# stevenlsw/reart

Measured on AMD Instinct MI355X. Metric: relaxation-loop iterations/sec, higher is better.
Workload: dtype f32; 1 GPU; synthetic T=20 x N=4096, P=20, Chamfer+flow, full iteration, one instance/GPU; frames=20, points=4096, parts=20, flow=True, graph=True, steps_per_graph=20, graph_replays=1, eager_steps=0, parallelism=instances x1, instances_per_gpu=1

## Files before the change

reart_amd/csrc/internal.h:

```cpp
#pragma once
#include "common.h"

struct BaseFwdArgs {
    const float *cano;
    const float *W1, *b1, *W2, *p6d, *pt;
    const float *gumbel;
    const float *tau_ptr;
    const int64_t *iter_ptr;
    uint64_t seed;
    float tau;
    int N, P, B, H, Npad;
    float *out;
    float *out_soa;
    int64_t *seg_part;
    float *trans_list;
    float *yT;
    float *hT;
    int *hard_idx;
    float *rt_table;
    float *boxes;
    int pts;
};

struct BaseBwdArgs {
    const float *cano, *W2, *p6d, *pt;
    const float *yT, *hT;
    const float *W1, *b1;
    const int *hard_idx;
    const float *tau_ptr;
    float tau;
    const float *G;
    const float *rt_table;
    const float *gpf;
    int cano_idx;
    int N, P, B, H;
    int nchunk;
    int cpts;
    int dp_sep;
    float *partial;
    const float *step_next;
    float *step_cur;
    float *gW1, *gb1, *gW2, *g6d, *gt;
};

struct AdamSeg { float *p; const float *g; float *m; float *v; int n; float lr; };
struct AdamArgs { AdamSeg seg[8]; int nseg; float beta1, beta2, eps; const int64_t *step_ptr; int step; };

#define REART_BATCH_MAX 6
template <class A>
struct Batched { A a[REART_BATCH_MAX]; };
template <class A>
static inline Batched<A> reart_batched(const A *a, int K) {
    Batched<A> b = {};
    for (int k = 0; k < K && k < REART_BATCH_MAX; ++k) b.a[k] = a[k];
    return b;
}
int reart_base_forward_launch(const BaseFwdArgs *a, int K, hipStream_t st, int force_long);
struct FinalizeAdam {
    int enabled;
    float *W1, *b1, *W2, *p6d, *pt;
    float *m, *v;
    float seg_lr, trans_lr, beta1, beta2, eps;
    float weight_decay;
    const int64_t *step_ptr;
    const float *step;
};

struct StepBook {
    int enabled;
    const double *frame_loss; int n_frame_part;
    const double *flow_part; int n_flow_part;
    int64_t *iter; float *tau; float *losses;
    float *step_next;
    int ring, n_iter;
    float lambda_flow, fixed_tau, end_tau, start_tau, beta1, beta2, seg_lr, trans_lr;
    const double *assign_part; int n_assign_part;
    float *losses_assign;
};
int reart_base_backward_launch(const BaseBwdArgs *args, const FinalizeAdam *adam, const StepBook *book, void *const *workspaces,
                               size_t workspace_bytes, int K, hipStream_t st, int force_long);
int reart_base_forward_long_launch(const BaseFwdArgs *a, int K, hipStream_t st);
int reart_base_backward_long_launch(const BaseBwdArgs *a, int K, hipStream_t st);
int reart_base_bwd_long_tile(int P, int B, int H, int cpts, int *dp_sep, size_t *lds);
#ifdef __HIPCC__
__device__ __forceinline__ float reart_tau_schedule(long cur_iter, int n_iter, float end_t, float start_t) {
    const double c = cos(3.14159265358979323846 * (double)cur_iter / (double)n_iter);
    return (float)((double)end_t + ((double)start_t - (double)end_t) * (c + 1.0) * 0.5);
}
#endif
int reart_adam_ex(const AdamArgs &a, hipStream_t st);

#define PG_SLICES (256 / 12)
int reart_pose_grad_launch(const float *x, const int64_t *part, const float *G, int N, int P, int B, float *partial, hipStream_t st);
int reart_fk_backward_launch(const float *x, const int64_t *part, const float *G, int N, const int32_t *parent,
                             const int32_t *edge_of_part, const int32_t *order, int P, const float *axis, const float *moment,
                             const float *theta, const float *distance, int B, int E, const float *trans, const float *g_trans,
                             float *g_axis, float *g_moment, float *g_theta, float *g_distance, void *workspace,
                             size_t workspace_bytes, hipStream_t st);

int reart_knn_run(int njobs, const float *const *q, const float *const *t,
                  const int64_t *const *lenq, const int64_t *const *lent, int N, const int *P1,
                  const int *P2, int K, int euclidean, float *const *dists, int64_t *const *idx,
                  void *workspace, size_t workspace_bytes, hipStream_t st);

#define NN_BS 64
#define NN_UB 16
struct SoaJob {
    const float *src;
    const int64_t *len;
    float *dst;
    int P, Ppad;
};
struct SoaArgs {
    SoaJob job[2];
};

struct KnnJob {
    const float *q;
    const float *tsoa;
    const int64_t *lenq;
    const int64_t *lent;
    const float *q_alt;
    const int *qmap;
    const int *tlen;
    const float *boxes;
    const int *seed;
    const int *border;
    unsigned int *cost;
    int P1, P2, Ppad, L;
    int nqg;
    float *pd;
    int *pi;
    float *dists;
    int64_t *idx;
};
struct KnnArgs {
    KnnJob job[2];
    int N, S, K, euclidean;
    int items0;
    int items;
};

int reart_knn_launch_slices(const KnnArgs &a, int KK, hipStream_t st);
int reart_soa_launch(const SoaArgs &sa, int maxPpad, int N, int njobs, hipStream_t st);
int reart_knn_pick_split(long waves, int P2, int K);

size_t reart_knn_list_workspace_bytes(int N, int P1, int P2, int K);
int reart_knn_list_run(const float *q, const float *t, const int64_t *lenq, const int64_t *lent, int N, int P1,
                       int P2, int K, int euclidean, float *dists, int64_t *idx, void *workspace,
                       size_t workspace_bytes, hipStream_t st);
template <class T>
int reart_knn_anyd_run(const T *q, const T *t, const int64_t *lenq, const int64_t *lent, int N, int P1, int P2, int D,
                       int K, int euclidean, T *dists, int64_t *idx, void *workspace, size_t workspace_bytes,
                       hipStream_t st);
#ifndef NN_BOX
#define NN_BOX 16
#endif
int reart_boxes_launch(const float *soa, int N, int Ppad, float *boxes, hipStream_t st);
struct SearchArgs {
    KnnJob k1[2]; int n1;
    KnnJob k3;    int n3;
    int G;
    int per;
    int S1, S3;
    int sparse;
    int share;
    int interleave;
    int cloud_resident;
    int cloud_slices;
    int k_nqg;
    unsigned long long *prof;
    unsigned int *prof_pairs;
};
int reart_search_launch(const SearchArgs &a, hipStream_t st);
int reart_search_launch_batch(const SearchArgs *a, int K, hipStream_t st);
int reart_search_grid(int n1, int n3, int G);
int reart_search_grid_cloud(int n1, int n3, int G, int nqg, int slices);
int reart_search_workgroups(const SearchArgs &a);

#ifdef __HIPCC__
__device__ __forceinline__ void reart_top3_insert(float (&kd)[3], int (&ki)[3], float d, int j) {
    const bool l0 = (d < kd[0]) | ((d == kd[0]) & (j < ki[0]));
    const bool l1 = (d < kd[1]) | ((d == kd[1]) & (j < ki[1]));
    const bool l2 = (d < kd[2]) | ((d == kd[2]) & (j < ki[2]));
    kd[2] = l1 ? kd[1] : (l2 ? d : kd[2]);
    ki[2] = l1 ? ki[1] : (l2 ? j : ki[2]);
    kd[1] = l0 ? kd[0] : (l1 ? d : kd[1]);
    ki[1] = l0 ? ki[0] : (l1 ? j : ki[1]);
    kd[0] = l0 ? d : kd[0];
    ki[0] = l0 ? j : ki[0];
}
#endif

struct GridBuildArgs {
    const float *pts;
    const int *offsets;
    int N;
    int stride;
    float *gx, *gy, *gz;
    int *gorig;
    int *cell_start;
    float *meta;
    int *scratch;
};

struct GridQueryArgs {
    const float *q;
    const float *q_alt;
    const int *qmap;
    int nq, E, stride, euclid_unused;
    const float *gx, *gy, *gz;
    const int *gorig, *cell_start;
    const float *meta;
    float *od;
    int *oi;
};

size_t reart_grid_bytes(int E, int stride);
void reart_grid_layout(void *mem, int E, int stride, GridBuildArgs *b);
int reart_grid_build_launch(const GridBuildArgs &b, int E, hipStream_t st);
int reart_grid_query_launch(const GridQueryArgs &q, int K, hipStream_t st);
```

reart_amd/csrc/prune.hip:

```cpp
#include "common.h"
#include "internal.h"
#include <math.h>
#include <string.h>

typedef float f2 __attribute__((ext_vector_type(2)));
#define PR_SMAX 4
#define PR_QCAP 640
#define PR_WPE 6
#define PR_LDS_WAVE_BYTES (64 * 4 + 64 * 16 + 3 * 64 * 8 + PR_QCAP * 4)

#ifdef REART_PRUNE_STATS
__device__ unsigned long long g_prune_stats[8];
extern "C" int reart_debug_prune_stats(unsigned long long *out, int reset) {
    if (hipMemcpyFromSymbol(out, HIP_SYMBOL(g_prune_stats), sizeof(g_prune_stats)) != hipSuccess) return REART_ERR_LAUNCH;
    if (reset) { unsigned long long z[8] = {0}; (void)hipMemcpyToSymbol(HIP_SYMBOL(g_prune_stats), z, sizeof(z)); }
    return REART_OK;
}
#define PRUNE_STAT(k, v) do { if ((threadIdx.x & 63) == 0) atomicAdd(&g_prune_stats[k], (unsigned long long)(v)); } while (0)
#else
#define PRUNE_STAT(k, v) do { } while (0)
#endif
#ifdef REART_PRUNE_PHASE
__device__ unsigned long long g_prune_phase[8];
extern "C" int reart_debug_prune_phase(unsigned long long *out, int reset) {
    if (hipMemcpyFromSymbol(out, HIP_SYMBOL(g_prune_phase), sizeof(g_prune_phase)) != hipSuccess) return REART_ERR_LAUNCH;
    if (reset) { unsigned long long z[8] = {0}; (void)hipMemcpyToSymbol(HIP_SYMBOL(g_prune_phase), z, sizeof(z)); }
    return REART_OK;
}
#define PH_DECL unsigned long long ph_t = __builtin_amdgcn_s_memtime(), ph_acc[7] = {0, 0, 0, 0, 0, 0, 0}
#define PH(k) do { const unsigned long long n_ = __builtin_amdgcn_s_memtime(); ph_acc[k] += n_ - ph_t; ph_t = n_; } while (0)
#define PH_FLUSH(from, to) do { if ((threadIdx.x & 63) == 0) for (int k_ = from; k_ <= to; ++k_) atomicAdd(&g_prune_phase[k_], ph_acc[k_]); } while (0)
#else
#define PH_DECL do { } while (0)
#define PH(k) do { } while (0)
#define PH_FLUSH(from, to) do { } while (0)
#endif

#define PR_WORK(w) ((unsigned)(w) << 20)

#define PR_DPP_OP(NAME, OP, CTRLTXT)                                                                              \
    __device__ __forceinline__ float NAME(float v) {                                                              \
        float r;                                                                                                  \
        asm("s_nop 1\n\t" OP " %0, %1, %1 " CTRLTXT " row_mask:0xf bank_mask:0xf" : "=v"(r) : "v"(v));            \
        return r;                                                                                                 \
    }
PR_DPP_OP(pr_min_q1, "v_min_f32_dpp", "quad_perm:[1,0,3,2]")
PR_DPP_OP(pr_min_q2, "v_min_f32_dpp", "quad_perm:[2,3,0,1]")
PR_DPP_OP(pr_min_hm, "v_min_f32_dpp", "row_half_mirror")
PR_DPP_OP(pr_min_rm, "v_min_f32_dpp", "row_mirror")
PR_DPP_OP(pr_max_q1, "v_max_f32_dpp", "quad_perm:[1,0,3,2]")
PR_DPP_OP(pr_max_q2, "v_max_f32_dpp", "quad_perm:[2,3,0,1]")
PR_DPP_OP(pr_max_hm, "v_max_f32_dpp", "row_half_mirror")
PR_DPP_OP(pr_max_rm, "v_max_f32_dpp", "row_mirror")
__device__ __forceinline__ float pr_row16_min(float v) { return pr_min_rm(pr_min_hm(pr_min_q2(pr_min_q1(v)))); }
__device__ __forceinline__ float pr_row16_max(float v) { return pr_max_rm(pr_max_hm(pr_max_q2(pr_max_q1(v)))); }

__device__ __forceinline__ float rl(float v, int lane) {
    return __int_as_float(__builtin_amdgcn_readlane(__float_as_int(v), lane));
}

__device__ __forceinline__ float box_lb(float lo0, float lo1, float lo2, float hi0, float hi1, float hi2,
                                        float qlo0, float qlo1, float qlo2, float qhi0, float qhi1, float qhi2) {
    const float ex = fmaxf(fmaxf(lo0 - qhi0, qlo0 - hi0), 0.f);
    const float ey = fmaxf(fmaxf(lo1 - qhi1, qlo1 - hi1), 0.f);
    const float ez = fmaxf(fmaxf(lo2 - qhi2, qlo2 - hi2), 0.f);
    return (ex * ex + ey * ey) + ez * ez;
}

template <int KK, bool LDSV, int QCAP, bool BOXL>
__device__ __forceinline__ void knn_pruned_wave(const KnnJob &jb, const int S, const int sparse, const int b, const int g,
                                                const int s, const float *cloud, const int cstride, const float *boxes_p,
                                                float *s_tg, float *s_qc, unsigned int *s_q, float *s_bb, const int share, float *s_xthr,
                                                unsigned long long *s_key, float &qx_o, float &qy_o, float &qz_o,
                                                float (&bm)[KK], int (&bb)[KK], int &work_o, unsigned int &pairs_o) {
    struct { int S, sparse; } a = {S, sparse};
    const int lane = threadIdx.x & 63;
    PH_DECL;

    const int i = g * NN_BS + lane;
    const int ic = i < jb.P1 ? i : jb.P1 - 1;
    const int qb = jb.qmap ? jb.qmap[b] : b;
    const float *qp = (qb < 0 ? jb.q_alt : jb.q + (size_t)qb * jb.P1 * 3) + (size_t)ic * 3;
    const float qx = qp[0], qy = qp[1], qz = qp[2];
    const f2 qx2 = {qx, qx}, qy2 = {qy, qy}, qz2 = {qz, qz};

    const float *tx = cloud;
    const float *ty = tx + cstride;
    const float *tz = ty + cstride;
    const int n2 = jb.tlen ? jb.tlen[b] : jb.P2;
    const int nbox = (n2 + NN_BOX - 1) / NN_BOX;
    const float *bx = boxes_p;

    float thr = 0.f;
    unsigned int wp = 0u;
    {
        const int *sd = jb.seed + ((size_t)b * jb.P1 + ic) * KK;
        int sj[KK];
        bool ok = true;
#pragma unroll
        for (int k = 0; k < KK; ++k) {
            sj[k] = sd[k];
            ok = ok && sj[k] >= 0 && sj[k] < n2;
#pragma unroll
            for (int k2 = 0; k2 < k; ++k2) ok = ok && sj[k] != sj[k2];
        }
        constexpr bool SCR_JOINT = BOXL;
        constexpr bool SCR_FITS = (384 + QCAP + (SCR_JOINT ? 384 : 0)) >= KK * 3 * 64;
        if (SCR_FITS && share) {
            float *s_scr = (float *)s_key;
#pragma unroll
            for (int k = 0; k < KK; ++k) {
                const int j = ok ? sj[k] : 0;
                s_scr[(3 * k + 0) * 64 + lane] = ok ? tx[j] : INFINITY;
                s_scr[(3 * k + 1) * 64 + lane] = ok ? ty[j] : INFINITY;
                s_scr[(3 * k + 2) * 64 + lane] = ok ? tz[j] : INFINITY;
            }
            thr = INFINITY;
            const float *row = s_scr + (lane & 48);
            const bool split = s_xthr != nullptr && a.S > 1;
            const int c0 = split ? 2 * s : 0, cstep = split ? 2 * a.S : 2;
            wp = 64u * KK * 2u * (unsigned)((16 - c0 + cstep - 1) / cstep);
#pragma unroll 1
            for (int c = c0; c < 16; c += cstep) {
                f2 far = {0.f, 0.f};
#pragma unroll
                for (int k = 0; k < KK; ++k) {
                    const f2 dx = qx2 - *(const f2 *)(row + (3 * k + 0) * 64 + c);
                    const f2 dy = qy2 - *(const f2 *)(row + (3 * k + 1) * 64 + c);
                    const f2 dz = qz2 - *(const f2 *)(row + (3 * k + 2) * 64 + c);
                    const f2 d = (dx * dx + dy * dy) + dz * dz;
                    far = f2{fmaxf(far.x, d.x), fmaxf(far.y, d.y)};
                }
                thr = fminf(thr, fminf(far.x, far.y));
            }
            if (split) {
                s_xthr[64 * s + lane] = thr;
                __syncthreads();
                for (int t = 0; t < a.S; ++t) thr = fminf(thr, s_xthr[64 * t + lane]);
            }
            if (!(qx == qx && qy == qy && qz == qz)) thr = INFINITY;
        } else {
#pragma unroll
            for (int k = 0; k < KK; ++k) {
                const int j = ok ? sj[k] : 0;
                thr = fmaxf(thr, reart_sqdist3(qx, qy, qz, tx[j], ty[j], tz[j]));
            }
            wp = 64u * KK;
            if (!ok || !(thr >= 0.f)) thr = INFINITY;
        }
    }

    const float gl0 = pr_row16_min(qx), gl1 = pr_row16_min(qy), gl2 = pr_row16_min(qz);
    const float gh0 = pr_row16_max(qx), gh1 = pr_row16_max(qy), gh2 = pr_row16_max(qz);
    const float gt = pr_row16_max(thr);
    float G[4][7];
#pragma unroll
    for (int q = 0; q < 4; ++q) {
        G[q][0] = rl(gl0, 16 * q); G[q][1] = rl(gl1, 16 * q); G[q][2] = rl(gl2, 16 * q);
        G[q][3] = rl(gh0, 16 * q); G[q][4] = rl(gh1, 16 * q); G[q][5] = rl(gh2, 16 * q);
        G[q][6] = rl(gt, 16 * q);
    }

#pragma unroll
    for (int k = 0; k < KK; ++k) { bm[k] = INFINITY; bb[k] = -1; }
    const float *tx_g = tx;
    wp |= PR_WORK(16);

    const int queue_max = a.sparse;
    int qcnt = 0;
    ((float4 *)s_qc)[lane] = make_float4(qx, qy, qz, 0.f);
    if (KK == 1) s_key[lane] = ~0ull;
    else { s_key[lane] = ~0ull; s_key[64 + lane] = ~0ull; s_key[128 + lane] = ~0ull; }
    auto drain_queue = [&]() {
        for (int e0 = 0; e0 < qcnt; e0 += 64) {
            wp += PR_WORK(6);
            const int e = e0 + lane;
            const bool valid = e < qcnt;
            const unsigned ent = s_q[valid ? e : e0];
            const int ql = (int)(ent & 63u), j0 = (int)(ent >> 6) * NN_BOX;
            wp += (unsigned)__builtin_popcountll(__ballot(valid)) * NN_BOX;
            const float4 qc = ((const float4 *)s_qc)[ql];
            const float *rx = tx_g, *ry = tx_g + cstride, *rz = tx_g + 2 * (size_t)cstride;
            const f2 cx = {qc.x, qc.x}, cy = {qc.y, qc.y}, cz = {qc.z, qc.z};
            float mh[2] = {INFINITY, INFINITY};
#pragma unroll 1
            for (int hf = 0; hf < 2; ++hf) {
                float4 X[2], Y[2], Z[2];
#pragma unroll
                for (int u = 0; u < 2; ++u) {
                    const unsigned ob = 4u * ((unsigned)j0 + 8u * hf + 4u * u);
                    X[u] = *(const float4 *)((const char *)rx + ob);
                    Y[u] = *(const float4 *)((const char *)ry + ob);
                    Z[u] = *(const float4 *)((const char *)rz + ob);
                }
                float m = INFINITY;
#pragma unroll
                for (int u = 0; u < 2; ++u) {
                    const f2 dxa = cx - f2{X[u].x, X[u].y}, dya = cy - f2{Y[u].x, Y[u].y}, dza = cz - f2{Z[u].x, Z[u].y};
                    const f2 dxb = cx - f2{X[u].z, X[u].w}, dyb = cy - f2{Y[u].z, Y[u].w}, dzb = cz - f2{Z[u].z, Z[u].w};
                    const f2 da = (dxa * dxa + dya * dya) + dza * dza;
                    const f2 db = (dxb * dxb + dyb * dyb) + dzb * dzb;
                    m = fminf(fminf(m, fminf(da.x, da.y)), fminf(db.x, db.y));
                }
                if (hf == 0) mh[0] = m; else mh[1] = m;
            }
            if (KK == 1) {
                const float m = fminf(mh[0], mh[1]);
                const unsigned long long key = ((unsigned long long)__float_as_uint(m) << 32) | (unsigned)(j0 + (mh[1] < mh[0] ? 8 : 0));
                if (valid) atomicMin(&s_key[ql], key);
            } else if (valid) {
#pragma unroll
                for (int h = 0; h < 2; ++h) {
                    unsigned long long key = ((unsigned long long)__float_as_uint(mh[h]) << 32) | (unsigned)(j0 + 8 * h);
#pragma unroll
                    for (int lv = 0; lv < 3; ++lv) {
                        const unsigned long long old = atomicMin(&s_key[64 * lv + ql], key);
                        key = old > key ? old : key;
                    }
                }
            }
        }
        qcnt = 0;
        if (KK == 1) {
            const unsigned long long k = s_key[lane];
            const float m = __uint_as_float((unsigned)(k >> 32));
            const int blk = (int)(unsigned)k;
            if (k != ~0ull && ((m < bm[0]) || (m == bm[0] && blk < bb[0]))) { bm[0] = m; bb[0] = blk; }
            thr = fminf(thr, bm[0]);
            s_key[lane] = ~0ull;
        } else {
            float kd[3];
            int ki[3];
#pragma unroll
            for (int c = 0; c < 3; ++c) { kd[c] = bm[c]; ki[c] = bb[c] >= 0 ? bb[c] : 0x7fffffff; }
#pragma unroll
            for (int c = 0; c < 3; ++c) {
                const unsigned long long k = s_key[64 * c + lane];
                s_key[64 * c + lane] = ~0ull;
                if (k != ~0ull) reart_top3_insert(kd, ki, __uint_as_float((unsigned)(k >> 32)), (int)(unsigned)k);
            }
#pragma unroll
            for (int c = 0; c < 3; ++c) { bm[c] = kd[c]; bb[c] = ki[c] == 0x7fffffff ? -1 : ki[c]; }
            thr = fminf(thr, bm[KK - 1]);
        }
    };
    const int per = 64 * a.S;
    PH(0);
    for (int base = 0; base < nbox; base += per) {
        const int bid = base + lane * a.S + s;
        bool pass = false;
        float lo0 = INFINITY, lo1 = INFINITY, lo2 = INFINITY, hi0 = INFINITY, hi1 = INFINITY, hi2 = INFINITY;
        if (bid < nbox) {
            const float4 A = *(const float4 *)(bx + (size_t)bid * 8);
            const float4 Bv = *(const float4 *)(bx + (size_t)bid * 8 + 4);
            lo0 = A.x; lo1 = A.y; lo2 = A.z; hi0 = A.w; hi1 = Bv.x; hi2 = Bv.y;
            if (BOXL) {
                float *o = s_bb + 6 * lane;
                o[0] = lo0; o[1] = lo1; o[2] = lo2; o[3] = hi0; o[4] = hi1; o[5] = hi2;
            }
            const f2 bl0 = {lo0, lo0}, bl1 = {lo1, lo1}, bl2 = {lo2, lo2}, bh0 = {hi0, hi0}, bh1 = {hi1, hi1}, bh2 = {hi2, hi2};
#pragma unroll
            for (int q = 0; q < 4; q += 2) {
                const f2 ql0 = {G[q][0], G[q + 1][0]}, ql1 = {G[q][1], G[q + 1][1]}, ql2 = {G[q][2], G[q + 1][2]};
                const f2 qh0 = {G[q][3], G[q + 1][3]}, qh1 = {G[q][4], G[q + 1][4]}, qh2 = {G[q][5], G[q + 1][5]};
                const f2 a0 = bl0 - qh0, c0 = ql0 - bh0, a1 = bl1 - qh1, c1 = ql1 - bh1, a2 = bl2 - qh2, c2 = ql2 - bh2;
                const f2 e0 = {fmaxf(fmaxf(a0.x, c0.x), 0.f), fmaxf(fmaxf(a0.y, c0.y), 0.f)};
                const f2 e1 = {fmaxf(fmaxf(a1.x, c1.x), 0.f), fmaxf(fmaxf(a1.y, c1.y), 0.f)};
                const f2 e2 = {fmaxf(fmaxf(a2.x, c2.x), 0.f), fmaxf(fmaxf(a2.y, c2.y), 0.f)};
                const f2 lb = (e0 * e0 + e1 * e1) + e2 * e2;
                pass = pass || (lb.x <= G[q][6]) || (lb.y <= G[q + 1][6]);
            }
        }
        unsigned long long mask = __ballot(pass);
        PH(1);
        PRUNE_STAT(KK == 1 ? 0 : 3, 0);
        if (KK == 1) PRUNE_STAT(1, __builtin_popcountll(mask));
        if (KK == 1) PRUNE_STAT(3, __builtin_popcountll(__ballot(thr == INFINITY)));
        auto scan_box = [&](const int bit) {
            wp += PR_WORK(5) | (64u * NN_BOX);
            if (KK == 1) PRUNE_STAT(2, 1);
            const int j0 = (base + bit * a.S + s) * NN_BOX;
            if (!LDSV) {
                const int l = lane < 48 ? lane : 47;
                const float v = tx_g[(size_t)(l >> 4) * cstride + j0 + (l & 15)];
                if (lane < 48) s_tg[lane] = v;
            }
            const float *tx = LDSV ? tx_g : s_tg - j0;
            const float *ty = tx + (LDSV ? cstride : 16), *tz = ty + (LDSV ? cstride : 16);
            if (KK == 1) {
                float mh[2] = {INFINITY, INFINITY};
#pragma unroll
                for (int u = 0; u < NN_BOX; u += 2) {
                    const f2 dx = qx2 - *(const f2 *)(tx + j0 + u);
                    const f2 dy = qy2 - *(const f2 *)(ty + j0 + u);
                    const f2 dz = qz2 - *(const f2 *)(tz + j0 + u);
                    const f2 d = (dx * dx + dy * dy) + dz * dz;
                    mh[u >> 3] = fminf(fminf(mh[u >> 3], d.x), d.y);
                }
                const float m = fminf(mh[0], mh[1]);
                if (m < bm[0]) { bm[0] = m; bb[0] = j0 + (mh[1] < mh[0] ? 8 : 0); }
                thr = fminf(thr, m);
            } else {
                constexpr int UBK = 8;
#pragma unroll
                for (int h = 0; h < NN_BOX; h += UBK) {
                    float m = INFINITY;
#pragma unroll
                    for (int u = 0; u < UBK; u += 2) {
                        const f2 dx = qx2 - *(const f2 *)(tx + j0 + h + u);
                        const f2 dy = qy2 - *(const f2 *)(ty + j0 + h + u);
                        const f2 dz = qz2 - *(const f2 *)(tz + j0 + h + u);
                        const f2 d = (dx * dx + dy * dy) + dz * dz;
                        m = fminf(fminf(m, d.x), d.y);
                    }
#pragma unroll
                    for (int c = KK - 1; c >= 0; --c) {
                        const int cp = c > 0 ? c - 1 : 0;
                        const bool lt_prev = (c > 0) && (m < bm[cp]);
                        const bool lt_cur = m < bm[c];
                        bm[c] = lt_prev ? bm[cp] : (lt_cur ? m : bm[c]);
                        bb[c] = lt_prev ? bb[cp] : (lt_cur ? j0 + h : bb[c]);
                    }
                }
                thr = fminf(thr, bm[KK - 1]);
            }
        };
        auto enqueue_box = [&](const int bit, const unsigned long long need, const bool nd, const int nneed) {
            wp += PR_WORK(1);
            if (KK == 1) PRUNE_STAT(2, 1);
            const int bid = base + bit * a.S + s;
            const int rank = __builtin_amdgcn_mbcnt_hi((unsigned)(need >> 32), __builtin_amdgcn_mbcnt_lo((unsigned)need, 0u));
            if (nd) s_q[qcnt + rank] = ((unsigned)bid << 6) | (unsigned)lane;
            qcnt += nneed;
        };
        while (mask) {
            unsigned long long cm = mask;
            mask = 0ull;
            while (cm) {
            const int bA = __builtin_ctzll(cm);
            cm &= cm - 1;
            const bool hasB = cm != 0;
            const int bB = hasB ? __builtin_ctzll(cm) : bA;
            if (hasB) cm &= cm - 1;
            f2 L0, L1, L2, H0, H1, H2;
            if (BOXL) {
                const float *pA = s_bb + 6 * bA, *pB = s_bb + 6 * bB;
                L0 = f2{pA[0], pB[0]}; L1 = f2{pA[1], pB[1]}; L2 = f2{pA[2], pB[2]};
                H0 = f2{pA[3], pB[3]}; H1 = f2{pA[4], pB[4]}; H2 = f2{pA[5], pB[5]};
            } else {
                L0 = f2{rl(lo0, bA), rl(lo0, bB)}; L1 = f2{rl(lo1, bA), rl(lo1, bB)}; L2 = f2{rl(lo2, bA), rl(lo2, bB)};
                H0 = f2{rl(hi0, bA), rl(hi0, bB)}; H1 = f2{rl(hi1, bA), rl(hi1, bB)}; H2 = f2{rl(hi2, bA), rl(hi2, bB)};
            }
            const f2 a0 = L0 - qx2, c0 = qx2 - H0, a1 = L1 - qy2, c1 = qy2 - H1, a2 = L2 - qz2, c2 = qz2 - H2;
            const f2 e0 = {fmaxf(fmaxf(a0.x, c0.x), 0.f), fmaxf(fmaxf(a0.y, c0.y), 0.f)};
            const f2 e1 = {fmaxf(fmaxf(a1.x, c1.x), 0.f), fmaxf(fmaxf(a1.y, c1.y), 0.f)};
            const f2 e2 = {fmaxf(fmaxf(a2.x, c2.x), 0.f), fmaxf(fmaxf(a2.y, c2.y), 0.f)};
            const f2 lb = (e0 * e0 + e1 * e1) + e2 * e2;
            wp += PR_WORK(2);
            PH(2);
#pragma unroll 1
            for (int h = 0; h < (hasB ? 2 : 1); ++h) {
                const float lbh = h ? lb.y : lb.x;
#ifdef REART_PRUNE_STATS
                if (KK == 1) {
                    const int nl = __builtin_popcountll(__ballot(lbh <= thr));
                    if (nl) PRUNE_STAT(nl == 1 ? 4 : (nl < 4 ? 5 : (nl < 8 ? 6 : 7)), 1);
                }
#endif
                const bool nd = lbh <= thr;
                const unsigned long long need = __ballot(nd);
                if (need) {
                    const int nneed = __builtin_popcountll(need);
                    if (nneed <= queue_max) {
                        enqueue_box(h ? bB : bA, need, nd, nneed);
                        PH(4);
                        if (qcnt > QCAP - 64) { drain_queue(); PH(5); }
                    } else {
                        scan_box(h ? bB : bA);
                        PH(3);
                    }
                }
            }
            }
        }
    }

    PH(2);
    if (qcnt > 0) drain_queue();
    PH(5);
    PH_FLUSH(0, 5);
    qx_o = qx; qy_o = qy; qz_o = qz;
    work_o = (int)(wp >> 20); pairs_o = wp & 0xFFFFFu;
}


template <bool BATCH>
__global__ __launch_bounds__(64 * PR_SMAX, PR_WPE) void knn_group_kernel(Batched<SearchArgs> ab) {
    const SearchArgs &a = ab.a[BATCH ? blockIdx.y : 0];
    extern __shared__ __attribute__((aligned(16))) unsigned char s_dyn[];
#define PARK_M(t) ((float *)(s_dyn + (size_t)(t) * PR_LDS_WAVE_BYTES + 64 * 4 + 64 * 16))
#define PARK_B(t) ((int *)(s_dyn + (size_t)(t) * PR_LDS_WAVE_BYTES + 64 * 4 + 64 * 16 + 3 * 64 * 4))
    __shared__ unsigned int s_wk[PR_SMAX][2];
    __shared__ float s_xthr[PR_SMAX][64];
    __shared__ unsigned int s_ticket;
    __shared__ unsigned long long s_t0;
    if (threadIdx.x == 0) { s_ticket = 0u; s_t0 = a.prof ? wall_clock64() : 0ull; }
    __syncthreads();
    const int L = blockIdx.x, x = L & 7, r = L >> 3;
    const int s = threadIdx.x >> 6, lane = threadIdx.x & 63;
    const unsigned long long t0 = s_t0;
    const int items1 = a.n1 * a.per, items3 = a.n3 * a.per;
    const int mixed = (a.n1 == 2 && a.n3) ? 3 * a.per : 0;
    int kind, idx;
    if (r < mixed) {
        const int q = r / 3, rr = r - 3 * q;
        kind = rr < 2 ? 1 : 3;
        idx = rr < 2 ? 2 * q + rr : q;
    } else {
        const int d1 = mixed ? 2 * a.per : 0, d3 = mixed ? a.per : 0;
        const int v = r - mixed, left1 = items1 - d1;
        kind = v < left1 ? 1 : 3;
        idx = v < left1 ? d1 + v : d3 + (v - left1);
    }
    const int j = kind == 1 ? (a.n1 == 2 ? (idx & 1) : 0) : 0;
    const int p = kind == 1 ? (a.n1 == 2 ? (idx >> 1) : idx) : idx;
    const int pos = a.interleave ? p * 8 + x : x * a.per + p;
    const bool live = p < a.per && pos < a.G && (kind == 1 ? idx < items1 : idx < items3);
    if (!live) {
        if (a.prof && threadIdx.x == 0) { a.prof[2 * (size_t)L] = t0; a.prof[2 * (size_t)L + 1] = t0; a.prof_pairs[L] = 0u; }
        return;
    }
    const KnnJob &jb = kind == 1 ? a.k1[j] : a.k3;
    const int S = kind == 1 ? a.S1 : a.S3;
    if (s >= S) return;
    const int grp = jb.border ? jb.border[pos] : pos;
    const int b = grp / jb.nqg, g = grp - b * jb.nqg;
    float qx = 0.f, qy = 0.f, qz = 0.f;
    float bm[3] = {INFINITY, INFINITY, INFINITY};
    int bb[3] = {-1, -1, -1};
    int work = 0;
    unsigned int pairs = 0u;
    {
        unsigned char *wl = s_dyn + (size_t)s * PR_LDS_WAVE_BYTES;
        float *s_tg = (float *)wl;
        float *s_qc = (float *)(wl + 64 * 4);
        unsigned long long *s_key = (unsigned long long *)(wl + 64 * 4 + 64 * 16);
        unsigned int *s_q = (unsigned int *)(wl + 64 * 4 + 64 * 16 + 3 * 64 * 8);
        static_assert(384 + PR_QCAP >= 3 * 3 * 64, "neighbour seeds of a K = 3 item: 9 x 64 floats in the result slots + the queue's space");
        static_assert(PR_QCAP >= 384 + 128, "box bounds of a coarse round + at least two drain steps of queue");
        float *s_bb = (float *)s_q;
        s_q += 384;
        constexpr int QC = PR_QCAP - 384;
        const float *cloud = jb.tsoa + (size_t)b * 3 * jb.Ppad;
        const float *boxes_p = jb.boxes + (size_t)b * (jb.Ppad / NN_BOX) * 8;
        if (kind == 1) {
            float m1[1]; int b1[1];
            knn_pruned_wave<1, false, QC, true>(jb, S, a.sparse, b, g, s, cloud, jb.Ppad, boxes_p, s_tg, s_qc, s_q, s_bb, a.share, a.share > 1 ? &s_xthr[0][0] : nullptr, s_key,
                                               qx, qy, qz, m1, b1, work, pairs);
            bm[0] = m1[0]; bb[0] = b1[0];
        } else {
            knn_pruned_wave<3, false, QC, true>(jb, S, a.sparse, b, g, s, cloud, jb.Ppad, boxes_p, s_tg, s_qc, s_q, s_bb, a.share, a.share > 1 ? &s_xthr[0][0] : nullptr, s_key,
                                               qx, qy, qz, bm, bb, work, pairs);
        }
    }
    if (S > 1) {
#pragma unroll
        for (int k = 0; k < 3; ++k) { PARK_M(s)[k * 64 + lane] = bm[k]; PARK_B(s)[k * 64 + lane] = bb[k]; }
        if (lane == 0) { s_wk[s][0] = (unsigned int)work; s_wk[s][1] = pairs; }
        __threadfence_block();
        int ticket = 0;
        if (lane == 0) ticket = (int)atomicAdd(&s_ticket, 1u);
        ticket = __builtin_amdgcn_readfirstlane(ticket);
#ifdef REART_PRUNE_PHASE
        if (lane == 0) atomicAdd(&g_prune_phase[7], 1ull);
#endif
        if (ticket != S - 1) return;
        __threadfence_block();
        work = 0; pairs = 0u;
        for (int t = 0; t < S; ++t) { work += (int)s_wk[t][0]; pairs += s_wk[t][1]; }
#pragma unroll
        for (int k = 0; k < 3; ++k) { bm[k] = PARK_M(0)[k * 64 + lane]; bb[k] = PARK_B(0)[k * 64 + lane]; }
    }
    const int i = g * NN_BS + lane;
    const float *tx = jb.tsoa + (size_t)b * 3 * jb.Ppad, *ty = tx + jb.Ppad, *tz = ty + jb.Ppad;
    if (kind == 1) {
        float m = bm[0];
        int blk = bb[0];
        for (int t = 1; t < S; ++t) {
            const float mt = PARK_M(t)[lane];
            const int bt = PARK_B(t)[lane];
            const bool take = bt >= 0 && ((mt < m) || (mt == m && (blk < 0 || bt < blk)));
            m = take ? mt : m; blk = take ? bt : blk;
        }
        int bi = 0x7fffffff;
        if (blk >= 0) {
#pragma unroll
            for (int u = NN_BOX / 2 - 1; u >= 0; --u) {
                const float d = reart_sqdist3(qx, qy, qz, tx[blk + u], ty[blk + u], tz[blk + u]);
                if (d == m) bi = blk + u;
            }
        }
        pairs += 64u * (NN_BOX / 2);
        if (i < jb.P1) {
            const size_t o = (size_t)b * jb.P1 + i;
            jb.pd[o] = m; jb.pi[o] = bi;
        }
    } else {
        float kd[3] = {INFINITY, INFINITY, INFINITY};
        int ki[3] = {0x7fffffff, 0x7fffffff, 0x7fffffff};
#pragma unroll
        for (int k = 0; k < 3; ++k) reart_top3_insert(kd, ki, bm[k], bb[k] >= 0 ? bb[k] : 0x7fffffff);
        for (int t = 1; t < S; ++t) {
#pragma unroll
            for (int k = 0; k < 3; ++k) {
                const int bt = PARK_B(t)[k * 64 + lane];
                reart_top3_insert(kd, ki, PARK_M(t)[k * 64 + lane], bt >= 0 ? bt : 0x7fffffff);
            }
        }
        if (i < jb.P1) {
            const size_t o = ((size_t)b * jb.P1 + i) * 3;
#pragma unroll
            for (int k = 0; k < 3; ++k) { jb.pd[o + k] = kd[k]; jb.pi[o + k] = kd[k] < INFINITY ? ki[k] : -1; }
        }
    }
    if (lane == 0) {
        if (jb.cost) jb.cost[pos] = (unsigned int)work;
        if (a.prof) {
            a.prof[2 * (size_t)L] = t0; a.prof[2 * (size_t)L + 1] = wall_clock64();
            a.prof_pairs[L] = pairs;
        }
    }
}

#define PC_WAVES 16
#define PC_QCAP 256
#define PC_WAVE_BYTES (64 * 16 + 3 * 64 * 8 + PC_QCAP * 4)
__global__ __launch_bounds__(64 * PC_WAVES) void knn_cloud_kernel(SearchArgs a) {
    extern __shared__ __attribute__((aligned(16))) unsigned char s_dyn[];
    const int L = blockIdx.x, w = threadIdx.x >> 6, lane = threadIdx.x & 63;
    unsigned long long t0 = 0ull;
    if (a.prof && threadIdx.x == 0) t0 = wall_clock64();
    const int njobs = a.n1 + a.n3;
    const int jsel = L % njobs;
    const int rest = L / njobs;
    const int B = a.G / a.k_nqg;
    const int b = rest % B, blk = rest / B;
    const int kind = jsel < a.n1 ? 1 : 3;
    const KnnJob &jb = kind == 1 ? a.k1[jsel] : a.k3;
    const int S = a.cloud_slices, gpw = PC_WAVES / S;
    const int Ppad = jb.Ppad, nboxp = Ppad / NN_BOX;
    float *cl = (float *)s_dyn;
    float *bxs = cl + 3 * (size_t)Ppad;
    {
        const float4 *src = (const float4 *)(jb.tsoa + (size_t)b * 3 * Ppad);
        float4 *dst = (float4 *)cl;
        const int n4 = 3 * Ppad / 4;
        for (int e = threadIdx.x; e < n4; e += 64 * PC_WAVES) dst[e] = src[e];
        const float4 *sb = (const float4 *)(jb.boxes + (size_t)b * nboxp * 8);
        float4 *db = (float4 *)bxs;
        for (int e = threadIdx.x; e < 2 * nboxp; e += 64 * PC_WAVES) db[e] = sb[e];
    }
    __syncthreads();
    const int g = blk * gpw + w / S, sl = w % S;
    unsigned int pairs = 0u;
    int work = 0;
    unsigned char *wbase = s_dyn + (size_t)(3 * Ppad + 8 * nboxp) * 4;
    unsigned long long *s_key = (unsigned long long *)(wbase + (size_t)w * PC_WAVE_BYTES + 64 * 16);
    float qx = 0.f, qy = 0.f, qz = 0.f;
    float bm[3] = {INFINITY, INFINITY, INFINITY};
    int bb[3] = {-1, -1, -1};
    if (g < jb.nqg) {
        unsigned char *wl = wbase + (size_t)w * PC_WAVE_BYTES;
        float *s_qc = (float *)wl;
        unsigned int *s_q = (unsigned int *)(wl + 64 * 16 + 3 * 64 * 8);
        if (kind == 1) {
            float m1[1]; int b1[1];
            knn_pruned_wave<1, true, PC_QCAP, false>(jb, S, a.sparse, b, g, sl, cl, Ppad, bxs, nullptr, s_qc, s_q, nullptr, a.share, nullptr, s_key, qx, qy, qz,
                                              m1, b1, work, pairs);
            bm[0] = m1[0]; bb[0] = b1[0];
        } else {
            knn_pruned_wave<3, true, PC_QCAP, false>(jb, S, a.sparse, b, g, sl, cl, Ppad, bxs, nullptr, s_qc, s_q, nullptr, a.share, nullptr, s_key, qx, qy, qz,
                                              bm, bb, work, pairs);
        }
        if (S > 1 && sl > 0) {
#pragma unroll
            for (int k = 0; k < 3; ++k)
                s_key[64 * k + lane] = bb[k] >= 0 ? (((unsigned long long)__float_as_uint(bm[k]) << 32) | (unsigned)bb[k]) : ~0ull;
            if (lane == 0) { s_key[192] = (unsigned long long)(unsigned)work; s_key[193] = (unsigned long long)pairs; }
        }
    }
    if (S > 1) __syncthreads();
    if (g < jb.nqg && sl == 0) {
        for (int t = 1; t < S; ++t) {
            const unsigned long long *ok = (const unsigned long long *)(wbase + (size_t)(w + t) * PC_WAVE_BYTES + 64 * 16);
            work += (int)(unsigned)ok[192]; pairs += (unsigned)ok[193];
            if (kind == 1) {
                const unsigned long long k = ok[lane];
                const float m = __uint_as_float((unsigned)(k >> 32));
                const int bt = (int)(unsigned)k;
                if (k != ~0ull && ((m < bm[0]) || (m == bm[0] && (bb[0] < 0 || bt < bb[0])))) { bm[0] = m; bb[0] = bt; }
            } else {
                float kd[3];
                int ki[3];
#pragma unroll
                for (int c = 0; c < 3; ++c) { kd[c] = bm[c]; ki[c] = bb[c] >= 0 ? bb[c] : 0x7fffffff; }
#pragma unroll
                for (int c = 0; c < 3; ++c) {
                    const unsigned long long k = ok[64 * c + lane];
                    if (k != ~0ull) reart_top3_insert(kd, ki, __uint_as_float((unsigned)(k >> 32)), (int)(unsigned)k);
                }
#pragma unroll
                for (int c = 0; c < 3; ++c) { bm[c] = kd[c]; bb[c] = ki[c] == 0x7fffffff ? -1 : ki[c]; }
            }
        }
        const int i = g * NN_BS + lane;
        if (kind == 1) {
            int bi = 0x7fffffff;
            if (bb[0] >= 0) {
                const float *tx = cl, *ty = cl + Ppad, *tz = cl + 2 * (size_t)Ppad;
#pragma unroll
                for (int u = NN_BOX / 2 - 1; u >= 0; --u) {
                    const float d = reart_sqdist3(qx, qy, qz, tx[bb[0] + u], ty[bb[0] + u], tz[bb[0] + u]);
                    if (d == bm[0]) bi = bb[0] + u;
                }
            }
            pairs += 64u * (NN_BOX / 2);
            if (i < jb.P1) {
                const size_t o = (size_t)b * jb.P1 + i;
                jb.pd[o] = bm[0]; jb.pi[o] = bi;
            }
        } else if (i < jb.P1) {
            const size_t o = ((size_t)b * jb.P1 + i) * 3;
#pragma unroll
            for (int k = 0; k < 3; ++k) { jb.pd[o + k] = bm[k]; jb.pi[o + k] = bm[k] < INFINITY ? bb[k] : -1; }
        }
        if (lane == 0 && jb.cost) jb.cost[b * jb.nqg + g] = (unsigned int)work;
    } else {
        pairs = 0u;
    }
    if (a.prof) {
        __shared__ unsigned int s_pairs[PC_WAVES];
        if (lane == 0) s_pairs[w] = pairs;
        __syncthreads();
        if (threadIdx.x == 0) {
            unsigned int tot = 0u;
            for (int k = 0; k < PC_WAVES; ++k) tot += s_pairs[k];
            a.prof[2 * (size_t)L] = t0; a.prof[2 * (size_t)L + 1] = wall_clock64();
            a.prof_pairs[L] = tot;
        }
    }
}

static size_t search_cloud_lds(const SearchArgs &a) {
    int Ppad = 0;
    for (int j = 0; j < a.n1; ++j) Ppad = a.k1[j].Ppad > Ppad ? a.k1[j].Ppad : Ppad;
    if (a.n3) Ppad = a.k3.Ppad > Ppad ? a.k3.Ppad : Ppad;
    const size_t need = (size_t)(3 * Ppad + 8 * (Ppad / NN_BOX)) * 4 + (size_t)PC_WAVES * PC_WAVE_BYTES + 256;
    return need <= 152 * 1024 ? need : 0;
}

static int search_check(SearchArgs &a) {
    if (a.n1 < 0 || a.n1 > 2 || a.n3 < 0 || a.n3 > 1 || a.n1 + a.n3 == 0 || a.G < 1) return REART_ERR_INVALID_ARG;
    if ((a.n1 && (a.S1 < 1 || a.S1 > PR_SMAX)) || (a.n3 && (a.S3 < 1 || a.S3 > PR_SMAX))) return REART_ERR_INVALID_ARG;
    for (int j = 0; j < a.n1; ++j)
        if (!a.k1[j].boxes || !a.k1[j].seed || !a.k1[j].pd || !a.k1[j].pi) return REART_ERR_INVALID_ARG;
    if (a.n3 && (!a.k3.boxes || !a.k3.seed || !a.k3.pd || !a.k3.pi)) return REART_ERR_INVALID_ARG;
    a.per = reart_div_up(a.G, 8);
    a.k_nqg = a.n1 ? a.k1[0].nqg : a.k3.nqg;
    return REART_OK;
}

int reart_search_launch(const SearchArgs &a_in, hipStream_t st) {
    SearchArgs a = a_in;
    const int rc = search_check(a);
    if (rc != REART_OK) return rc;
    const size_t cl_lds = a.cloud_resident ? search_cloud_lds(a) : 0;
    a.cloud_slices = (a.cloud_slices == 1 || a.cloud_slices == 2 || a.cloud_slices == 4 || a.cloud_slices == 8) ? a.cloud_slices : 4;
    if (cl_lds) {
        if (hipFuncSetAttribute((const void *)knn_cloud_kernel, hipFuncAttributeMaxDynamicSharedMemorySize, 152 * 1024) != hipSuccess)
            return REART_ERR_LAUNCH;
        hipLaunchKernelGGL(knn_cloud_kernel, dim3(reart_search_grid_cloud(a.n1, a.n3, a.G, a.k_nqg, a.cloud_slices)), dim3(64 * PC_WAVES),
                           cl_lds, st, a);
        REART_CHECK_LAUNCH();
        return REART_OK;
    }
    return reart_search_launch_batch(&a, 1, st);
}
int reart_search_launch_batch(const SearchArgs *ak, int K, hipStream_t st) {
    if (K < 1 || K > REART_BATCH_MAX) return REART_ERR_INVALID_ARG;
    Batched<SearchArgs> ab = {};
    for (int k = 0; k < K; ++k) {
        ab.a[k] = ak[k];
        const int rc = search_check(ab.a[k]);
        if (rc != REART_OK) return rc;
        const SearchArgs &a = ab.a[k], &a0 = ab.a[0];
        if (a.n1 != a0.n1 || a.n3 != a0.n3 || a.G != a0.G || a.S1 != a0.S1 || a.S3 != a0.S3) return REART_ERR_INVALID_ARG;
    }
    const SearchArgs &a = ab.a[0];
    const int S = (a.n1 ? a.S1 : 0) > (a.n3 ? a.S3 : 0) ? a.S1 : a.S3;
    const size_t lds = (size_t)S * PR_LDS_WAVE_BYTES;
    if (K == 1) hipLaunchKernelGGL(knn_group_kernel<false>, dim3(reart_search_grid(a.n1, a.n3, a.G)), dim3(64 * S), lds, st, ab);
    else hipLaunchKernelGGL(knn_group_kernel<true>, dim3(reart_search_grid(a.n1, a.n3, a.G), K), dim3(64 * S), lds, st, ab);
    REART_CHECK_LAUNCH();
    return REART_OK;
}
int reart_search_workgroups(const SearchArgs &a) {
    const int nqg = a.n1 ? a.k1[0].nqg : a.k3.nqg;
    const int cs = (a.cloud_slices == 1 || a.cloud_slices == 2 || a.cloud_slices == 4 || a.cloud_slices == 8) ? a.cloud_slices : 4;
    if (a.cloud_resident && search_cloud_lds(a)) return reart_search_grid_cloud(a.n1, a.n3, a.G, nqg, cs);
    return reart_search_grid(a.n1, a.n3, a.G);
}
int reart_search_grid(int n1, int n3, int G) { return 8 * (n1 + n3) * reart_div_up(G, 8); }
int reart_search_grid_cloud(int n1, int n3, int G, int nqg, int slices) {
    return (n1 + n3) * (G / nqg) * reart_div_up(nqg, PC_WAVES / slices);
}

template <int KK>
__global__ __launch_bounds__(256) void knn_warm_finish_kernel(KnnArgs a) {
    const KnnJob jb = a.job[0];
    const int b = blockIdx.y, i = blockIdx.x * 256 + threadIdx.x;
    if (i >= jb.P1) return;
    float kd[KK];
    int ki[KK];
#pragma unroll
    for (int k = 0; k < KK; ++k) { kd[k] = INFINITY; ki[k] = 0x7fffffff; }
    auto insert = [&](float d, int j) {
#pragma unroll
        for (int s = KK - 1; s >= 0; --s) {
            const int sp = s > 0 ? s - 1 : 0;
            const bool lp = (s > 0) && ((d < kd[sp]) | ((d == kd[sp]) & (j < ki[sp])));
            const bool lc = (d < kd[s]) | ((d == kd[s]) & (j < ki[s]));
            kd[s] = lp ? kd[sp] : (lc ? d : kd[s]);
            ki[s] = lp ? ki[sp] : (lc ? j : ki[s]);
        }
    };
    {
        const size_t o = ((size_t)b * jb.P1 + i) * KK;
#pragma unroll
        for (int k = 0; k < KK; ++k) {
            const float d = jb.pd[o + k];
            const int q = jb.pi[o + k];
            insert(d, (d < INFINITY && q >= 0) ? q : 0x7fffffff);
        }
    }
    if (KK > 1) {
        const float *qp = jb.q + ((size_t)b * jb.P1 + i) * 3;
        const float qx = qp[0], qy = qp[1], qz = qp[2];
        const float *tx = jb.tsoa + (size_t)b * 3 * jb.Ppad, *ty = tx + jb.Ppad, *tz = ty + jb.Ppad;
        int blk[KK];
#pragma unroll
        for (int k = 0; k < KK; ++k) { blk[k] = kd[k] < INFINITY ? ki[k] : -1; kd[k] = INFINITY; ki[k] = 0x7fffffff; }
#pragma unroll
        for (int c = 0; c < KK; ++c) {
            if (blk[c] < 0) continue;
            for (int u = 0; u < 8; ++u) {
                const int jj = blk[c] + u;
                const float d = reart_sqdist3(qx, qy, qz, tx[jj], ty[jj], tz[jj]);
                insert(d, d < INFINITY ? jj : 0x7fffffff);
            }
        }
    }
    const int n2 = jb.P2;
    const int valid = KK < n2 ? KK : n2;
#pragma unroll
    for (int k = 0; k < KK; ++k) {
        const bool ok = k < valid && ki[k] != 0x7fffffff;
        const size_t o = ((size_t)b * jb.P1 + i) * KK + k;
        jb.dists[o] = ok ? kd[k] : 0.0f;
        jb.idx[o] = ok ? (int64_t)ki[k] : (int64_t)0;
        ((int *)jb.seed)[o] = ok ? ki[k] : -1;
    }
}

struct WarmPlan { int S, Ppad; size_t o_soa, o_box, o_pd, o_pi, total; };
static int warm_plan(int N, int P1, int P2, int K, WarmPlan *p) {
    if (N < 0 || P1 < 0 || P2 < 0 || (K != 1 && K != 3)) return REART_ERR_INVALID_ARG;
    p->S = 4;
    while (p->S > 1 && reart_div_up(P2, p->S) < 64) p->S -= 1;
    p->Ppad = (int)reart_align_up((size_t)(P2 > 0 ? P2 : 1), NN_BOX);
    reart_arena ws;
    p->o_soa = ws.take_bytes(sizeof(float) * 3 * (size_t)N * p->Ppad);
    p->o_box = ws.take_bytes(sizeof(float) * 8 * (size_t)N * (p->Ppad / NN_BOX));
    p->o_pd = ws.take_bytes(sizeof(float) * (size_t)N * P1 * K);
    p->o_pi = ws.take_bytes(sizeof(int) * (size_t)N * P1 * K);
    p->total = ws.off;
    return REART_OK;
}

extern "C" size_t reart_knn_points_warm_workspace_bytes(int N, int P1, int P2, int K) {
    WarmPlan p;
    return warm_plan(N, P1, P2, K, &p) == REART_OK ? p.total : 0;
}

extern "C" int reart_knn_points_idx_warm(const float *p1, const float *p2, int N, int P1, int P2, int K,
                                         int32_t *seed, float *dists, int64_t *idx, void *workspace,
                                         size_t workspace_bytes, void *stream) {
    WarmPlan p;
    int rc = warm_plan(N, P1, P2, K, &p);
    if (rc != REART_OK) return rc;
    if (N == 0 || P1 == 0) return REART_OK;
    if (!p1 || !p2 || !seed || !dists || !idx || P2 < 1) return REART_ERR_INVALID_ARG;
    if (!workspace || workspace_bytes < p.total) return REART_ERR_INVALID_ARG;
    hipStream_t st = (hipStream_t)stream;
    char *ws = (char *)workspace;
    SoaArgs sa = {};
    for (int j = 0; j < 2; ++j) {
        sa.job[j].src = p2; sa.job[j].len = nullptr; sa.job[j].dst = (float *)(ws + p.o_soa);
        sa.job[j].P = P2; sa.job[j].Ppad = p.Ppad;
    }
    rc = reart_soa_launch(sa, p.Ppad, N, 1, st);
    if (rc != REART_OK) return rc;
    rc = reart_boxes_launch((const float *)(ws + p.o_soa), N, p.Ppad, (float *)(ws + p.o_box), st);
    if (rc != REART_OK) return rc;
    KnnArgs a = {};
    a.N = N; a.S = p.S; a.K = K; a.euclidean = 0;
    KnnJob &jb = a.job[0];
    jb.q = p1; jb.tsoa = (const float *)(ws + p.o_soa); jb.boxes = (const float *)(ws + p.o_box);
    jb.seed = seed; jb.P1 = P1; jb.P2 = P2; jb.Ppad = p.Ppad; jb.L = 0; jb.nqg = reart_div_up(P1, NN_BS);
    jb.pd = (float *)(ws + p.o_pd); jb.pi = (int *)(ws + p.o_pi); jb.dists = dists; jb.idx = idx;
    a.job[1] = jb;
    SearchArgs sr = {};
    sr.G = N * jb.nqg; sr.S1 = sr.S3 = p.S; sr.sparse = 40; sr.share = 2;
    if (K == 1) { sr.k1[0] = jb; sr.n1 = 1; } else { sr.k3 = jb; sr.n3 = 1; }
    rc = reart_search_launch(sr, st);
    if (rc != REART_OK) return rc;
    const dim3 fg(reart_div_up(P1, 256), N);
    if (K == 1) hipLaunchKernelGGL((knn_warm_finish_kernel<1>), fg, dim3(256), 0, st, a);
    else hipLaunchKernelGGL((knn_warm_finish_kernel<3>), fg, dim3(256), 0, st, a);
    REART_CHECK_LAUNCH();
    return REART_OK;
}
```

reart_amd/csrc/step.hip:

```cpp
#include "common.h"
#include "internal.h"
#include "blocksort.h"
#include "consumer_dev.h"
#include "flow_dev.h"
#include <math.h>
#include <string.h>

struct StepPlan {
    int S1, L1, Npad;
    int S3, Mpad;
    int nchunk, nparams;
    size_t o_ysoa, o_xsoa, o_rsoa, o_rlen, o_qmap;
    size_t o_pd0, o_pi0, o_pd1, o_pi1, o_pd3, o_pi3;
    size_t o_yT, o_hT, o_hard, o_rt, o_G, o_gpf, o_fx, o_floss, o_apart, o_fpart, o_grads, o_bwd;
    size_t o_bc;
    size_t o_ticket;
    size_t o_boxY, o_boxX, o_boxR;
    int keep_hT;
    int pruned;
    int W1, W3;
    int sparse;
    size_t o_seed3;
    size_t o_border;
    size_t o_cost;
    size_t o_prof, o_prof_pairs, o_prof_acc;
    size_t o_gridY, o_gridR;
    int gstrideY, gstrideR;
    size_t bwd_bytes, total;
};

#define FLOW_BS 256
#define CG_BS 1024
#define POST_FBS 512
#define CG_RANGE 1024
static_assert(CG_BS == CG_RANGE, "chamfer_grad_kernel: thread tid owns target r0 + tid");

static int step_plan(const reart_relax_config *c, StepPlan *p) {
    if (c->N <= 0 || c->P <= 0 || c->P > 32 || c->B <= 0 || c->H <= 0) return REART_ERR_INVALID_ARG;
    if (c->use_flow && (c->flow_k != 3 || c->M_max < 3)) return REART_ERR_UNSUPPORTED;
    const long waves1 = 2L * c->B * reart_div_up(c->N, NN_BS);
    p->pruned = (c->use_boxes && !c->use_grid && c->search_mode != 1) ? 1 : 0;
    p->W1 = (c->tune_slices >= 1 && c->tune_slices <= 4) ? c->tune_slices : 3;
    p->W3 = (c->tune_slices_flow >= 1 && c->tune_slices_flow <= 4) ? c->tune_slices_flow : p->W1;
    p->sparse = c->tune_sparse < 0 ? 0 : (c->tune_sparse == 0 ? 40 : (c->tune_sparse > 64 ? 64 : c->tune_sparse));
    p->S1 = p->pruned ? 1 : reart_knn_pick_split(waves1, c->N, 1);
    p->L1 = (int)reart_align_up((size_t)reart_div_up(c->N, p->S1), NN_BOX);
    p->Npad = p->L1 * p->S1;
    p->S3 = 1; p->Mpad = 0;
    if (c->use_flow) {
        const long waves3 = (long)c->B * reart_div_up(c->N, NN_BS);
        p->S3 = p->pruned ? 1 : reart_knn_pick_split(waves3, c->M_max, 3);
        p->Mpad = (int)reart_align_up((size_t)reart_div_up(c->M_max, p->S3), NN_BOX) * p->S3;
    }
    p->nchunk = reart_div_up(c->N, 64);
    p->nparams = 3 * c->H + c->H + c->P * c->H + 6 * c->B * c->P + 3 * c->B * c->P;
    reart_arena ws;
    const size_t BN = (size_t)c->B * c->N;
    p->o_ysoa = ws.take_bytes(sizeof(float) * 3 * c->B * (size_t)p->Npad);
    p->o_xsoa = ws.take_bytes(sizeof(float) * 3 * c->B * (size_t)p->Npad);
    p->o_rsoa = ws.take_bytes(sizeof(float) * 3 * c->B * (size_t)p->Mpad);
    p->o_rlen = ws.take_bytes(sizeof(int) * c->B);
    p->o_qmap = ws.take_bytes(sizeof(int) * (c->B + 1));
    p->o_pd0 = ws.take_bytes(sizeof(float) * p->S1 * BN);
    p->o_pi0 = ws.take_bytes(sizeof(int) * p->S1 * BN);
    p->o_pd1 = ws.take_bytes(sizeof(float) * p->S1 * BN);
    p->o_pi1 = ws.take_bytes(sizeof(int) * p->S1 * BN);
    p->o_pd3 = ws.take_bytes(c->use_flow ? sizeof(float) * p->S3 * BN * 3 : 0);
    p->o_pi3 = ws.take_bytes(c->use_flow ? sizeof(int) * p->S3 * BN * 3 : 0);
    p->o_yT = ws.take_bytes(sizeof(float) * (size_t)c->P * c->N);
    p->keep_hT = (c->tune_long > 0 || reart_base_path(c->P, c->B, c->H, 0) != 0 || reart_base_path(c->P, c->B, c->H, 1) != 0) ? 1 : 0;
    p->o_hT = ws.take_bytes(p->keep_hT ? sizeof(float) * (size_t)c->H * c->N : 0);
    p->o_hard = ws.take_bytes(sizeof(int) * (size_t)c->N);
    p->o_rt = ws.take_bytes(sizeof(float) * 12 * (size_t)c->B * c->P);
    p->o_G = ws.take_bytes(sizeof(float) * 3 * BN);
    p->o_gpf = ws.take_bytes(sizeof(float) * 3 * BN);
    p->o_fx = ws.take_bytes(sizeof(double));
    p->o_floss = ws.take_bytes(sizeof(double) * (size_t)c->B * reart_div_up(c->N, CG_RANGE));
    p->o_apart = ws.take_bytes(c->recon_with_assign ? sizeof(double) * (size_t)c->B * reart_div_up(c->N, CG_RANGE) : 0);
    p->o_fpart = ws.take_bytes(sizeof(double) * (size_t)c->B * reart_div_up(c->N, FLOW_BS));
    p->o_grads = ws.take_bytes(sizeof(float) * p->nparams);
    p->bwd_bytes = reart_base_backward_workspace_bytes(c->N, c->P, c->B, c->H);
    p->o_bwd = ws.take_bytes(p->bwd_bytes);
    p->o_bc = ws.take_bytes(8 * sizeof(float));
    p->o_ticket = ws.take_bytes(4 * sizeof(unsigned int));
    p->o_boxY = ws.take_bytes(sizeof(float) * 8 * (size_t)c->B * (p->Npad / NN_BOX));
    p->o_boxX = ws.take_bytes(sizeof(float) * 8 * (size_t)c->B * (p->Npad / NN_BOX));
    p->o_boxR = ws.take_bytes(sizeof(float) * 8 * (size_t)c->B * (p->Mpad / NN_BOX + 1));
    p->o_seed3 = ws.take_bytes((p->pruned && c->use_flow) ? sizeof(int) * BN * 3 : 0);
    const size_t G = (size_t)c->B * reart_div_up(c->N, NN_BS);
    p->o_border = ws.take_bytes(sizeof(int) * 3 * G);
    p->o_cost = ws.take_bytes(sizeof(unsigned int) * 3 * G);
    const size_t nprof = (c->profile && p->pruned) ? (size_t)reart_search_grid(2, 1, (int)G) : 0;
    p->o_prof = ws.take_bytes(sizeof(unsigned long long) * 2 * nprof);
    p->o_prof_pairs = ws.take_bytes(sizeof(unsigned int) * nprof);
    p->o_prof_acc = ws.take_bytes(sizeof(unsigned long long) * 4);
    p->gstrideY = (int)reart_align_up((size_t)c->N, 64);
    p->gstrideR = (int)reart_align_up((size_t)(c->M_max > 0 ? c->M_max : 1), 64);
    p->o_gridY = ws.take_bytes(c->use_grid ? reart_grid_bytes(c->B, p->gstrideY) : 0);
    p->o_gridR = ws.take_bytes((c->use_grid && c->use_flow) ? reart_grid_bytes(c->B, p->gstrideR) : 0);
    p->total = ws.off;
    return REART_OK;
}

extern "C" size_t reart_relax_workspace_bytes(const reart_relax_config *cfg) {
    StepPlan p;
    if (!cfg || step_plan(cfg, &p) != REART_OK) return 0;
    return p.total;
}

__global__ void relax_init_kernel(reart_relax_config c, const int *__restrict__ ref_off,
                                  int *__restrict__ rlen, int *__restrict__ qmap,
                                  int64_t *__restrict__ iter, float *__restrict__ tau,
                                  const float *__restrict__ pc_list, int *__restrict__ fx_bits,
                                  float *__restrict__ adam_step, int *__restrict__ seed3, int *__restrict__ border) {
    __shared__ float s_max[1024];
    const int t = threadIdx.x;
    if (seed3)
        for (size_t e = t; e < (size_t)c.B * c.N * 3; e += 1024) seed3[e] = (int)(e % 3);
    float mx = 0.f;
    for (size_t e = t; e < (size_t)c.B * c.N * 3; e += 1024) mx = fmaxf(mx, fabsf(pc_list[e]));
    s_max[t] = mx;
    __syncthreads();
    for (int o = 512; o >= 1; o >>= 1) {
        if (t < o) s_max[t] = fmaxf(s_max[t], s_max[t + o]);
        __syncthreads();
    }
    if (t == 0) {
        const double bound = 8.0 * (double)c.N * fmax((double)s_max[0], 1e-30);
        int bits = (int)floor(61.0 - log2(bound));
        fx_bits[0] = bits > 39 ? 39 : (bits < 0 ? 0 : bits);
    }
    if (t < c.B) {
        {
            const int nqg = (c.N + NN_BS - 1) / NN_BS, ng = c.B * nqg;
            for (int g = 0; g < nqg; ++g)
                for (int j = 0; j < 3; ++j) border[j * ng + t * nqg + g] = t * nqg + g;
        }
        qmap[t] = (t < c.cano_idx) ? t : (t == c.cano_idx ? -1 : t - 1);
        if (c.use_flow) rlen[t] = ref_off[t + 1] - ref_off[t];
    }
    if (t == 0) {
        const long it = (long)iter[0];
        tau[0] = c.fixed_tau > 0.f ? c.fixed_tau : reart_tau_schedule(it + 1, c.n_iter, c.end_tau, c.start_tau);
        const double bc1 = 1.0 - pow((double)c.beta1, (double)(it + 1));
        const double bc2 = sqrt(1.0 - pow((double)c.beta2, (double)(it + 1)));
        for (int s = 0; s < 8; s += 4) {
            adam_step[s] = (float)((double)c.seg_lr / bc1);
            adam_step[s + 1] = (float)((double)c.trans_lr / bc1);
            adam_step[s + 2] = (float)bc2;
            adam_step[s + 3] = 0.f;
        }
    }
}

__global__ __launch_bounds__(256) void ref_soa_kernel(const float *__restrict__ ref_loc,
                                                      const int *__restrict__ ref_off, int Mpad,
                                                      float *__restrict__ soa) {
    const int f = blockIdx.y, j = blockIdx.x * 256 + threadIdx.x;
    if (j >= Mpad) return;
    const int o = ref_off[f], m = ref_off[f + 1] - o;
    float x = INFINITY, y = INFINITY, z = INFINITY;
    if (j < m) {
        const float *p = ref_loc + 3 * ((size_t)o + j);
        x = p[0]; y = p[1]; z = p[2];
    }
    float *d = soa + (size_t)f * 3 * Mpad;
    d[j] = x; d[Mpad + j] = y; d[2 * (size_t)Mpad + j] = z;
}

extern "C" int reart_relax_prepare(const reart_relax_config *cfg, const reart_relax_buffers *bufs,
                                   void *workspace, size_t workspace_bytes, void *stream) {
    StepPlan p;
    if (!cfg || !bufs) return REART_ERR_INVALID_ARG;
    int rc = step_plan(cfg, &p);
    if (rc != REART_OK) return rc;
    if (!workspace || workspace_bytes < p.total) return REART_ERR_INVALID_ARG;
    if (!bufs->cano || !bufs->pc_list || !bufs->iter || !bufs->tau) return REART_ERR_INVALID_ARG;
    if (cfg->use_flow && (!bufs->ref_loc || !bufs->ref_flow || !bufs->ref_off)) return REART_ERR_INVALID_ARG;
    static_assert(REART_MAX_POSE_LEN <= 1024, "relax_init_kernel: one thread per frame");
    if (cfg->B > REART_MAX_POSE_LEN) return REART_ERR_UNSUPPORTED;
    char *ws = (char *)workspace;
    hipStream_t st = (hipStream_t)stream;
    SoaArgs sa = {};
    for (int j = 0; j < 2; ++j) {
        sa.job[j].src = bufs->pc_list; sa.job[j].len = nullptr;
        sa.job[j].dst = (float *)(ws + p.o_ysoa); sa.job[j].P = cfg->N; sa.job[j].Ppad = p.Npad;
    }
    rc = reart_soa_launch(sa, p.Npad, cfg->B, 1, st);
    if (rc != REART_OK) return rc;
    hipLaunchKernelGGL(relax_init_kernel, dim3(1), dim3(1024), 0, st, *cfg, bufs->ref_off,
                       (int *)(ws + p.o_rlen), (int *)(ws + p.o_qmap), bufs->iter, bufs->tau, bufs->pc_list,
                       (int *)(ws + p.o_fx), (float *)(ws + p.o_bc),
                       (p.pruned && cfg->use_flow) ? (int *)(ws + p.o_seed3) : nullptr, (int *)(ws + p.o_border));
    if (hipMemsetAsync(ws + p.o_ticket, 0, 4 * sizeof(unsigned int), st) != hipSuccess) return REART_ERR_LAUNCH;
    if (hipMemsetAsync(ws + p.o_prof_acc, 0, 4 * sizeof(unsigned long long), st) != hipSuccess) return REART_ERR_LAUNCH;
    if (p.pruned) {
        if (hipMemsetAsync(ws + p.o_pi0, 0, sizeof(int) * (size_t)cfg->B * cfg->N, st) != hipSuccess) return REART_ERR_LAUNCH;
        if (hipMemsetAsync(ws + p.o_pi1, 0, sizeof(int) * (size_t)cfg->B * cfg->N, st) != hipSuccess) return REART_ERR_LAUNCH;
    }
    rc = reart_boxes_launch((const float *)(ws + p.o_ysoa), cfg->B, p.Npad, (float *)(ws + p.o_boxY), st);
    if (rc != REART_OK) return rc;
    if (cfg->use_grid) {
        GridBuildArgs gb = {};
        reart_grid_layout(ws + p.o_gridY, cfg->B, p.gstrideY, &gb);
        gb.pts = bufs->pc_list; gb.offsets = nullptr; gb.N = cfg->N;
        rc = reart_grid_build_launch(gb, cfg->B, st);
        if (rc != REART_OK) return rc;
        if (cfg->use_flow) {
            GridBuildArgs gr = {};
            reart_grid_layout(ws + p.o_gridR, cfg->B, p.gstrideR, &gr);
            gr.pts = bufs->ref_loc; gr.offsets = bufs->ref_off; gr.N = cfg->M_max;
            rc = reart_grid_build_launch(gr, cfg->B, st);
            if (rc != REART_OK) return rc;
        }
    }
    if (cfg->use_flow)
    {
        hipLaunchKernelGGL(ref_soa_kernel, dim3(reart_div_up(p.Mpad, 256), cfg->B), dim3(256), 0, st,
                           bufs->ref_loc, bufs->ref_off, p.Mpad, (float *)(ws + p.o_rsoa));
        rc = reart_boxes_launch((const float *)(ws + p.o_rsoa), cfg->B, p.Mpad, (float *)(ws + p.o_boxR), st);
        if (rc != REART_OK) return rc;
    }
    REART_CHECK_LAUNCH();
    return REART_OK;
}

struct FlowArgs {
    const float *pd; const int *pi;
    const float *ref_flow; const int *ref_off; const int *qmap;
    const float *X; const float *cano;
    int N, B, S, euclidean, robust, cano_idx;
    int blocks;
    const float *rsoa; int Mpad;
    float smooth, lambda;
    float *gpf;
    double *part;
    int *seed_out;
};

template <int SL, int FBS>
__device__ __forceinline__ void flow_blend_body(const FlowArgs &a, const int bx, const int f, const int nbx) {
    __shared__ double s_red[FBS / REART_WAVE];
    const int n = bx * FBS + threadIdx.x;
    double term = 0.0;
    if (n < a.N) {
        constexpr int NU = SL == 1 ? 1 : 4;
        float kd[3] = {INFINITY, INFINITY, INFINITY};
        int ki[3] = {0x7fffffff, 0x7fffffff, 0x7fffffff};
        const size_t stride = (size_t)a.B * a.N * 3, o0 = ((size_t)f * a.N + n) * 3;
        const float *c0 = reart_complete_frame(a.X, a.cano, a.N, a.cano_idx, f) + 3 * (size_t)n;
        const float *c1 = reart_complete_frame(a.X, a.cano, a.N, a.cano_idx, f + 1) + 3 * (size_t)n;
        const float c0v[3] = {c0[0], c0[1], c0[2]}, c1v[3] = {c1[0], c1[1], c1[2]};
        const int roff = a.ref_off[f];
        for (int s0 = 0; s0 < (SL ? 1 : a.S); s0 += 4) {
            float e[NU][3];
            int q[NU][3];
#pragma unroll
            for (int u = 0; u < NU; ++u) {
                const bool ok = s0 + u < a.S;
                const size_t o = o0 + (size_t)(ok ? s0 + u : 0) * stride;
#pragma unroll
                for (int k = 0; k < 3; ++k) { e[u][k] = a.pd[o + k]; q[u][k] = a.pi[o + k]; }
                if (!ok) { e[u][0] = INFINITY; e[u][1] = INFINITY; e[u][2] = INFINITY; }
            }
#pragma unroll
            for (int u = 0; u < NU; ++u)
#pragma unroll
                for (int k = 0; k < 3; ++k)
                    reart_top3_insert(kd, ki, e[u][k], e[u][k] < INFINITY ? q[u][k] : 0x7fffffff);
        }
        if (a.blocks) {
            const float *tx = a.rsoa + (size_t)f * 3 * a.Mpad, *ty = tx + a.Mpad, *tz = ty + a.Mpad;
            int bb[3], nv[3];
#pragma unroll
            for (int cb = 0; cb < 3; ++cb) {
                bb[cb] = (kd[cb] < INFINITY) ? ki[cb] : -1;
                nv[cb] = bb[cb] < 0 ? 0 : 8;
            }
            reart_rescan3(c0v, tx, ty, tz, bb, nv, kd, ki);
        }
#pragma unroll
        for (int k = 0; k < 3; ++k) ki[k] = ki[k] == 0x7fffffff ? 0 : ki[k];
        if (a.seed_out) {
            int *so = a.seed_out + 3 * ((size_t)f * a.N + n);
            so[0] = ki[0]; so[1] = ki[1]; so[2] = ki[2];
        }
        const float *rf = a.ref_flow + 3 * (size_t)roff;
        float rfl[3][3];
#pragma unroll
        for (int k = 0; k < 3; ++k)
#pragma unroll
            for (int c = 0; c < 3; ++c) rfl[k][c] = rf[3 * (size_t)ki[k] + c];
        float w[3], wsum = 0.f, dmin = INFINITY, fmx = -INFINITY;
#pragma unroll
        for (int k = 0; k < 3; ++k) {
            float d = a.euclidean ? sqrtf(kd[k]) : kd[k];
            if (d < 1e-10f) d = 1e-10f;
            w[k] = 1.0f / d;
            wsum += w[k];
            dmin = fminf(dmin, d);
            fmx = fmaxf(fmx, (rfl[k][0] * rfl[k][0] + rfl[k][1] * rfl[k][1]) + rfl[k][2] * rfl[k][2]);
        }
        float gtf[3] = {0.f, 0.f, 0.f};
#pragma unroll
        for (int k = 0; k < 3; ++k) {
            const float wn = w[k] / wsum;
            gtf[0] += rfl[k][0] * wn; gtf[1] += rfl[k][1] * wn; gtf[2] += rfl[k][2] * wn;
        }
        const bool m = (dmin <= fmx) || (dmin <= 0.05f);
        float fl = 0.f, sm = 0.f;
        float *go = a.gpf + 3 * ((size_t)f * a.N + n);
#pragma unroll
        for (int c = 0; c < 3; ++c) {
            const float p = c1v[c] - c0v[c];
            const float d = p - gtf[c];
            fl += a.robust ? huber1(d) : d * d;
            sm += p * p;
            const float gf = a.robust ? huber1_grad(d) : 2.0f * d;
            go[c] = a.lambda * (m ? gf : a.smooth * (2.0f * p));
        }
        term = m ? (double)fl : (double)(a.smooth * sm);
    }
    term = reart_block_sum_d<FBS>(term, s_red);
    if (threadIdx.x == 0) a.part[(size_t)f * nbx + bx] = term;
}

struct CGradArgs {
    const float *X, *Y;
    const float *pd0; const int *pi0;
    const float *pd1; const int *pi1;
    const int *fx_bits;
    int N, B, S0, S1;
    float *G;
    double *loss_part;
    int *seed0, *seed1;
    const int *map;
    double *assign_part;
    float lambda;
};
template <int SL>
__device__ __forceinline__ void merge_slices(const float *__restrict__ pd, const int *__restrict__ pi, int S,
                                             size_t stride, size_t o0, int nmax, float &d, int &j) {
    d = INFINITY; j = 0x7fffffff;
    constexpr int NU = SL == 1 ? 1 : 4;
    for (int s0 = 0; s0 < (SL ? 1 : S); s0 += 4) {
        float e[NU];
        int q[NU];
#pragma unroll
        for (int u = 0; u < NU; ++u) {
            const size_t o = o0 + (size_t)(s0 + u < S ? s0 + u : S - 1) * stride;
            e[u] = pd[o]; q[u] = pi[o];
        }
#pragma unroll
        for (int u = 0; u < NU; ++u) {
            const bool l = (e[u] < d) | ((e[u] == d) & (q[u] < j));
            d = l ? e[u] : d; j = l ? q[u] : j;
        }
    }
    j = j < 0 ? 0 : (j >= nmax ? nmax - 1 : j);
}

template <int SL, bool AS>
__device__ __forceinline__ void chamfer_grad_body(const CGradArgs &a, const int bx, const int b, const int nbx) {
    __shared__ unsigned long long s_acc[CG_RANGE * 3];
    __shared__ double s_red[CG_BS / REART_WAVE];
    const int tid = threadIdx.x, N = a.N;
    const int r0 = bx * CG_RANGE;
    const float *x = a.X + (size_t)b * N * 3, *y = a.Y + (size_t)b * N * 3;
    const size_t stride = (size_t)a.B * N, ob = (size_t)b * N;
    for (int e = tid; e < CG_RANGE * 3; e += CG_BS) s_acc[e] = 0ull;
    const int io = r0 + tid, ioc = io < N ? io : N - 1;
    float d0;
    int j0;
    int am = -1;
    if (AS) am = a.map[ob + ioc];
    merge_slices<SL>(a.pd0, a.pi0, a.S0, stride, ob + ioc, N, d0, j0);
    const int sbits = a.fx_bits[0];
    float yn[3], xo[3];
#pragma unroll
    for (int k = 0; k < 3; ++k) { yn[k] = y[3 * j0 + k]; xo[k] = x[3 * ioc + k]; }
    const bool paired = AS && am >= 0 && am < N;
    float ya[3] = {0.f, 0.f, 0.f};
    if (AS) {
        const int amc = paired ? am : 0;
#pragma unroll
        for (int k = 0; k < 3; ++k) ya[k] = y[3 * amc + k];
    }
    __syncthreads();
    float d1own = 0.f;
    constexpr int IL = 4;
    for (int ib = tid; ib < N; ib += IL * CG_BS) {
        float d1[IL];
        int j1[IL];
#pragma unroll
        for (int u = 0; u < IL; ++u) {
            const int i = ib + u * CG_BS;
            merge_slices<SL>(a.pd1, a.pi1, a.S1, stride, ob + (i < N ? i : N - 1), N, d1[u], j1[u]);
        }
        float df[IL][3];
#pragma unroll
        for (int u = 0; u < IL; ++u) {
            const int i = ib + u * CG_BS;
            const int ic = i < N ? i : N - 1;
#pragma unroll
            for (int k = 0; k < 3; ++k) df[u][k] = x[3 * j1[u] + k] - y[3 * ic + k];
        }
#pragma unroll
        for (int u = 0; u < IL; ++u) {
            const int i = ib + u * CG_BS;
            if (i >= N) continue;
            if (i == io) {
                d1own = d1[u];
                if (a.seed1) a.seed1[ob + i] = j1[u];
            }
            const int jl = j1[u] - r0;
            if (jl >= 0 && jl < CG_RANGE) {
#pragma unroll
                for (int k = 0; k < 3; ++k)
                    atomicAdd(&s_acc[3 * jl + k], (unsigned long long)reart_fixed_from_float(df[u][k], sbits));
            }
        }
    }
    if (io < N && a.seed0) a.seed0[ob + io] = j0;
    __syncthreads();
    double term = 0.0, aterm = 0.0;
    if (io < N) {
        term = (double)(d0 + d1own);
        const double inv2 = 2.0 * exp2((double)-sbits);
        float *G = a.G + 3 * (ob + io);
        float sq = 0.f;
#pragma unroll
        for (int k = 0; k < 3; ++k) {
            const float gc = 2.0f * (xo[k] - yn[k]) + (float)((double)(long long)s_acc[3 * tid + k] * inv2);
            if (AS && paired) {
                const float d = xo[k] - ya[k];
                sq += d * d;
                G[k] = gc + a.lambda * (2.0f * d);
            } else {
                G[k] = gc;
            }
        }
        if (AS && paired) aterm = (double)sq;
    }
    term = reart_block_sum_d<CG_BS>(term, s_red);
    if (tid == 0) a.loss_part[(size_t)b * nbx + bx] = term;
    if (AS) {
        __syncthreads();
        aterm = reart_block_sum_d<CG_BS>(aterm, s_red);
        if (tid == 0) a.assign_part[(size_t)b * nbx + bx] = aterm * (double)a.lambda;
    }
}

template <int SL, bool BATCH, bool AS>
__global__ __launch_bounds__(CG_BS) void chamfer_grad_kernel(Batched<CGradArgs> ab) {
    chamfer_grad_body<SL, AS>(ab.a[BATCH ? blockIdx.z : 0], blockIdx.x, blockIdx.y, gridDim.x);
}
template <int SL, bool BATCH>
__global__ __launch_bounds__(FLOW_BS) void flow_blend_kernel(Batched<FlowArgs> ab) {
    flow_blend_body<SL, FLOW_BS>(ab.a[BATCH ? blockIdx.z : 0], blockIdx.x, blockIdx.y, gridDim.x);
}
struct OrderArgs {
    const unsigned int *cost[3];
    int *border[3];
    int groups;
    int per;
    const unsigned long long *prof; const unsigned int *prof_pairs; unsigned long long *prof_acc; int nprof;
};
#define ORD_MAX 4
__device__ __forceinline__ void order_body(const OrderArgs &o, const int j) {
    __shared__ unsigned int s_hist[8 * 256];
    const int tid = threadIdx.x;
    if (!o.cost[j] || o.groups > ORD_MAX * CG_BS) return;
    for (int e = tid; e < 8 * 256; e += CG_BS) s_hist[e] = 0u;
    __syncthreads();
    int old[ORD_MAX], bucket[ORD_MAX];
#pragma unroll
    for (int u = 0; u < ORD_MAX; ++u) {
        const int k = tid + u * CG_BS;
        old[u] = 0; bucket[u] = -1;
        if (k < o.groups) {
            const unsigned int c = o.cost[j][k] >> 5;
            old[u] = o.border[j][k];
            bucket[u] = (k / o.per) * 256 + 255 - (int)(c < 255u ? c : 255u);
            atomicAdd(&s_hist[bucket[u]], 1u);
        }
    }
    __syncthreads();
    for (int c0 = (tid >> 6); c0 < 8; c0 += CG_BS / 64) {
        const int l = tid & 63;
        unsigned int v[4], sum = 0u;
#pragma unroll
        for (int k = 0; k < 4; ++k) { v[k] = s_hist[c0 * 256 + 4 * l + k]; sum += v[k]; }
        unsigned int incl = sum;
#pragma unroll
        for (int off = 1; off < 64; off <<= 1) {
            const unsigned int t = __shfl_up(incl, off, 64);
            if (l >= off) incl += t;
        }
        unsigned int run = (unsigned int)(c0 * o.per) + (incl - sum);
#pragma unroll
        for (int k = 0; k < 4; ++k) { s_hist[c0 * 256 + 4 * l + k] = run; run += v[k]; }
    }
    __syncthreads();
#pragma unroll
    for (int u = 0; u < ORD_MAX; ++u)
        if (bucket[u] >= 0) o.border[j][atomicAdd(&s_hist[bucket[u]], 1u)] = old[u];
}
__device__ __forceinline__ void prof_body(const OrderArgs &o) {
    __shared__ unsigned long long s_lo[CG_BS / 64], s_hi[CG_BS / 64], s_sum[CG_BS / 64], s_busy[CG_BS / 64];
    const int tid = threadIdx.x;
    unsigned long long lo = ~0ull, hi = 0ull, sum = 0ull, busy = 0ull;
    for (int k = tid; k < o.nprof; k += CG_BS) {
        const unsigned long long a = o.prof[2 * (size_t)k], b = o.prof[2 * (size_t)k + 1];
        lo = a < lo ? a : lo; hi = b > hi ? b : hi; sum += o.prof_pairs[k]; busy += b - a;
    }
#pragma unroll
    for (int off = 32; off >= 1; off >>= 1) {
        const unsigned long long l2 = __shfl_xor(lo, off, 64), h2 = __shfl_xor(hi, off, 64), s2 = __shfl_xor(sum, off, 64);
        const unsigned long long b2 = __shfl_xor(busy, off, 64);
        lo = l2 < lo ? l2 : lo; hi = h2 > hi ? h2 : hi; sum += s2; busy += b2;
    }
    if ((tid & 63) == 0) { s_lo[tid >> 6] = lo; s_hi[tid >> 6] = hi; s_sum[tid >> 6] = sum; s_busy[tid >> 6] = busy; }
    __syncthreads();
    if (tid == 0) {
        for (int w = 1; w < CG_BS / 64; ++w) {
            lo = s_lo[w] < lo ? s_lo[w] : lo; hi = s_hi[w] > hi ? s_hi[w] : hi; sum += s_sum[w]; busy += s_busy[w];
        }
        o.prof_acc[0] += 1ull; o.prof_acc[1] += hi - lo; o.prof_acc[2] += sum; o.prof_acc[3] += busy;
    }
}
struct PostArgs { int nfx, nflow, ncx, nwork, norder; FlowArgs fl; CGradArgs cg; OrderArgs od; };
#ifdef REART_PHASE_CLOCK
__device__ unsigned long long g_post_ts[8];
extern "C" int reart_debug_post_clock(unsigned long long *out) {
    return hipMemcpyFromSymbol(out, HIP_SYMBOL(g_post_ts), sizeof(g_post_ts)) == hipSuccess ? REART_OK : REART_ERR_LAUNCH;
}
#define POST_TS(k) do { __syncthreads(); if (threadIdx.x == 0 && blockIdx.y == 0) g_post_ts[k] = __builtin_amdgcn_s_memtime(); } while (0)
#else
#define POST_TS(k) do { } while (0)
#endif
template <bool BATCH, bool AS>
__global__ __launch_bounds__(CG_BS) void post_kernel(Batched<PostArgs> ab) {
    const PostArgs &a = ab.a[BATCH ? blockIdx.y : 0];
    const int w = blockIdx.x;
    if (w < a.nflow) {
        if (threadIdx.x >= POST_FBS) return;
        if (w == 1) POST_TS(0);
        flow_blend_body<1, POST_FBS>(a.fl, w % a.nfx, w / a.nfx, a.nfx);
        if (w == 1) POST_TS(1);
    } else if (w < a.nwork) {
        if (w == a.nflow + 1) POST_TS(2);
        chamfer_grad_body<1, AS>(a.cg, (w - a.nflow) % a.ncx, (w - a.nflow) / a.ncx, a.ncx);
        if (w == a.nflow + 1) POST_TS(3);
    } else if (w < a.nwork + a.norder) {
        if (w == a.nwork) POST_TS(4);
        order_body(a.od, w - a.nwork);
        if (w == a.nwork) POST_TS(5);
    } else {
        POST_TS(6);
        prof_body(a.od);
        POST_TS(7);
    }
}

struct AssignArgs {
    const float *X, *Y;
    const int *map;
    int N, B;
    float lambda;
    float *G;
    double *loss_part;
};
__device__ __forceinline__ void assign_grad_body(const AssignArgs &a, int bx, int b, int gx) {
    __shared__ double s_red[CG_BS / REART_WAVE];
    const int i = bx * CG_BS + threadIdx.x, tid = threadIdx.x;
    double term = 0.0;
    if (i < a.N) {
        const size_t o = (size_t)b * a.N + i;
        const int m = a.map[o];
        float g[3] = {0.f, 0.f, 0.f};
        if (m >= 0 && m < a.N) {
            float sq = 0.f;
#pragma unroll
            for (int k = 0; k < 3; ++k) {
                const float d = a.X[3 * o + k] - a.Y[3 * ((size_t)b * a.N + m) + k];
                sq += d * d;
                g[k] = a.lambda * (2.0f * d);
            }
            term = (double)sq;
        }
#pragma unroll
        for (int k = 0; k < 3; ++k) a.G[3 * o + k] = g[k];
    }
    term = reart_block_sum_d<CG_BS>(term, s_red);
    if (tid == 0) a.loss_part[(size_t)b * gx + bx] = term * (double)a.lambda;
}
template <bool BATCH>
__global__ __launch_bounds__(CG_BS) void assign_grad_kernel(Batched<AssignArgs> ab) {
    assign_grad_body(ab.a[BATCH ? blockIdx.z : 0], blockIdx.x, blockIdx.y, gridDim.x);
}

#define MARK(k) do { if (ev) (void)hipEventRecord(ev[k], st); } while (0)

struct StepGeom {
    int pruned, grid;
    int flow;
    int merged;
    int has_search;
    int static_order;
    int has_fl, has_aa, has_cg;
    int fl_sl, cg_sl;
    int fgx, fgy, ncg, post_blocks, N, B;
    int long_model;
    int cg_assign;
};
struct StepLaunch {
    StepGeom g;
    BaseFwdArgs fa; SearchArgs sa; KnnArgs ka, k3; GridQueryArgs gq3, gq1; PostArgs pa;
    FlowArgs fl; AssignArgs aa; CGradArgs cg;
    BaseBwdArgs ba; FinalizeAdam ad; StepBook bk; void *ws_bwd; size_t bwd_bytes;
    int auto_s1, auto_s3;
    void *aux_stream, *ev_fork, *ev_join;
};

static int step_describe(const reart_relax_config *cfg, const reart_relax_buffers *bufs, void *workspace, size_t workspace_bytes,
                         bool forward_only, StepLaunch *out) {
    StepPlan p;
    if (!cfg || !bufs) return REART_ERR_INVALID_ARG;
    int rc = step_plan(cfg, &p);
    if (rc != REART_OK) return rc;
    if (!workspace || workspace_bytes < p.total) return REART_ERR_INVALID_ARG;
    if (!bufs->W1 || !bufs->b1 || !bufs->W2 || !bufs->p6d || !bufs->pt || !bufs->adam_m || !bufs->adam_v ||
        !bufs->pc_trans || !bufs->iter || !bufs->tau)
        return REART_ERR_INVALID_ARG;
    const reart_relax_config &c = *cfg;
    StepLaunch &L = *out;
    L = StepLaunch{};
    StepGeom &g = L.g;
    char *ws = (char *)workspace;
    const int N = c.N, B = c.B, P = c.P, H = c.H;
    float *G = (float *)(ws + p.o_G);
    g.N = N; g.B = B; g.pruned = p.pruned; g.grid = c.use_grid ? 1 : 0; g.flow = c.use_flow ? 1 : 0;
    g.long_model = c.tune_long > 0 ? 1 : 0;

    BaseFwdArgs &fa = L.fa;
    fa.cano = bufs->cano; fa.W1 = bufs->W1; fa.b1 = bufs->b1; fa.W2 = bufs->W2; fa.p6d = bufs->p6d;
    fa.pt = bufs->pt; fa.gumbel = bufs->gumbel; fa.tau_ptr = bufs->tau; fa.iter_ptr = bufs->iter;
    fa.seed = c.seed; fa.tau = 1.0f; fa.N = N; fa.P = P; fa.B = B; fa.H = H; fa.Npad = p.Npad;
    fa.out = bufs->pc_trans; fa.out_soa = (float *)(ws + p.o_xsoa); fa.seg_part = bufs->seg_part;
    fa.trans_list = bufs->trans_list; fa.yT = (float *)(ws + p.o_yT); fa.hT = p.keep_hT ? (float *)(ws + p.o_hT) : nullptr;
    fa.hard_idx = (int *)(ws + p.o_hard);
    fa.rt_table = (float *)(ws + p.o_rt);
    fa.boxes = c.use_boxes ? (float *)(ws + p.o_boxX) : nullptr;
    fa.pts = c.tune_fwd_pts;
    if (forward_only) return REART_OK;
    if (c.use_assign && !bufs->assign_map) return REART_ERR_INVALID_ARG;

    const int nqg = reart_div_up(N, NN_BS);
    const int *qmap = (const int *)(ws + p.o_qmap);
    KnnArgs &ka = L.ka, &k3 = L.k3;
    ka.N = B; ka.S = p.S1; ka.K = 1; ka.euclidean = 0;
    for (int j = 0; j < 2; ++j) {
        KnnJob &kj = ka.job[j];
        kj.q = j == 0 ? bufs->pc_trans : bufs->pc_list;
        kj.tsoa = (const float *)(ws + (j == 0 ? p.o_ysoa : p.o_xsoa));
        kj.P1 = N; kj.P2 = N; kj.Ppad = p.Npad; kj.L = p.L1; kj.nqg = nqg;
        kj.pd = (float *)(ws + (j == 0 ? p.o_pd0 : p.o_pd1));
        kj.pi = (int *)(ws + (j == 0 ? p.o_pi0 : p.o_pi1));
        kj.boxes = c.use_boxes ? (const float *)(ws + (j == 0 ? p.o_boxY : p.o_boxX)) : nullptr;
        kj.seed = p.pruned ? kj.pi : nullptr;
        kj.border = (const int *)(ws + p.o_border) + (size_t)j * B * nqg;
        kj.cost = p.pruned ? (unsigned int *)(ws + p.o_cost) + (size_t)j * B * nqg : nullptr;
    }
    ka.items0 = B * nqg * p.S1; ka.items = 2 * ka.items0;
    if (c.use_flow) {
        k3.N = B; k3.S = p.S3; k3.K = 3; k3.euclidean = 0;
        KnnJob &kj = k3.job[0];
        kj.q = bufs->pc_trans; kj.q_alt = bufs->cano; kj.qmap = qmap;
        kj.tsoa = (const float *)(ws + p.o_rsoa); kj.tlen = (const int *)(ws + p.o_rlen);
        kj.boxes = c.use_boxes ? (const float *)(ws + p.o_boxR) : nullptr;
        kj.P1 = N; kj.P2 = c.M_max; kj.Ppad = p.Mpad; kj.L = p.Mpad / p.S3; kj.nqg = nqg;
        kj.pd = (float *)(ws + p.o_pd3); kj.pi = (int *)(ws + p.o_pi3);
        kj.seed = p.pruned ? (const int *)(ws + p.o_seed3) : nullptr;
        kj.border = (const int *)(ws + p.o_border) + 2 * (size_t)B * nqg;
        kj.cost = p.pruned ? (unsigned int *)(ws + p.o_cost) + 2 * (size_t)B * nqg : nullptr;
        k3.job[1] = kj;
        k3.items0 = B * nqg * p.S3; k3.items = k3.items0;
    }
    const bool both = c.use_assign && c.recon_with_assign;
    const bool chamfer = !c.use_assign || both;
    g.cg_assign = both ? 1 : 0;
    const bool merged = p.pruned && c.use_flow && chamfer;
    g.merged = merged ? 1 : 0;
    L.aux_stream = bufs->aux_stream; L.ev_fork = bufs->ev_fork; L.ev_join = bufs->ev_join;

    int search_wgs = 0, S3 = p.S3, S0 = p.S1;
    if (p.pruned) {
        SearchArgs &sa = L.sa;
        sa.G = B * nqg; sa.S1 = p.W1; sa.S3 = p.W3; sa.sparse = p.sparse; sa.share = c.tune_share < 0 ? 0 : (c.tune_share == 1 ? 1 : 2); sa.interleave = c.tune_xcd > 0 ? 0 : 1;
        sa.cloud_resident = c.tune_cloud > 0 ? 1 : 0; sa.cloud_slices = c.tune_cloud > 0 ? c.tune_cloud : 0;
        if (chamfer) { sa.k1[0] = ka.job[0]; sa.k1[1] = ka.job[1]; sa.n1 = 2; }
        if (c.use_flow) { sa.k3 = k3.job[0]; sa.n3 = 1; }
        if (c.profile && merged) {
            sa.prof = (unsigned long long *)(ws + p.o_prof); sa.prof_pairs = (unsigned int *)(ws + p.o_prof_pairs);
        }
        L.auto_s1 = c.tune_slices == 0; L.auto_s3 = c.tune_slices_flow == 0;
        if (sa.n1 + sa.n3 > 0) {
            search_wgs = reart_search_workgroups(sa);
            g.static_order = search_wgs != reart_search_grid(sa.n1, sa.n3, sa.G);
            g.has_search = 1;
        }
    } else if (c.use_grid) {
        if (c.use_flow) {
            GridBuildArgs gr = {};
            reart_grid_layout(ws + p.o_gridR, B, p.gstrideR, &gr);
            GridQueryArgs &gq = L.gq3;
            gq.q = bufs->pc_trans; gq.q_alt = bufs->cano; gq.qmap = qmap; gq.nq = N; gq.E = B; gq.stride = p.gstrideR;
            gq.gx = gr.gx; gq.gy = gr.gy; gq.gz = gr.gz; gq.gorig = gr.gorig; gq.cell_start = gr.cell_start;
            gq.meta = gr.meta; gq.od = (float *)(ws + p.o_pd3); gq.oi = (int *)(ws + p.o_pi3);
            S3 = 1;
        }
        if (chamfer) {
            GridBuildArgs gy = {};
            reart_grid_layout(ws + p.o_gridY, B, p.gstrideY, &gy);
            GridQueryArgs &gq = L.gq1;
            gq.q = bufs->pc_trans; gq.nq = N; gq.E = B; gq.stride = p.gstrideY; gq.gx = gy.gx; gq.gy = gy.gy; gq.gz = gy.gz;
            gq.gorig = gy.gorig; gq.cell_start = gy.cell_start; gq.meta = gy.meta;
            gq.od = (float *)(ws + p.o_pd0); gq.oi = (int *)(ws + p.o_pi0);
            S0 = 1;
            ka.job[0] = ka.job[1];
            ka.items = ka.items0;
        }
    }
    int nfp = 0;
    FlowArgs &fl = L.fl;
    if (c.use_flow) {
        fl.pd = (const float *)(ws + p.o_pd3); fl.pi = (const int *)(ws + p.o_pi3); fl.ref_flow = bufs->ref_flow;
        fl.ref_off = bufs->ref_off; fl.qmap = qmap; fl.X = bufs->pc_trans; fl.cano = bufs->cano; fl.N = N; fl.B = B;
        fl.blocks = c.use_grid ? 0 : 1; fl.rsoa = (const float *)(ws + p.o_rsoa); fl.Mpad = p.Mpad;
        fl.S = S3; fl.euclidean = c.euclidean; fl.robust = c.robust; fl.cano_idx = c.cano_idx;
        fl.smooth = c.smooth_weight; fl.lambda = c.lambda_flow;
        fl.gpf = (float *)(ws + p.o_gpf); fl.part = (double *)(ws + p.o_fpart);
        fl.seed_out = p.pruned ? (int *)(ws + p.o_seed3) : nullptr;
        g.fgx = reart_div_up(N, merged ? POST_FBS : FLOW_BS); g.fgy = B;
        nfp = g.fgx * g.fgy;
        g.has_fl = merged ? 0 : 1; g.fl_sl = fl.S == 1 ? 1 : (fl.S <= 4 ? 4 : 0);
    }
    g.ncg = reart_div_up(N, CG_RANGE);
    if (!chamfer) {
        AssignArgs &aa = L.aa;
        aa.X = bufs->pc_trans; aa.Y = bufs->pc_list; aa.map = bufs->assign_map; aa.N = N; aa.B = B;
        aa.lambda = c.lambda_assign; aa.G = G; aa.loss_part = (double *)(ws + p.o_floss);
        g.has_aa = 1;
    } else {
        CGradArgs &cg = L.cg;
        cg.X = bufs->pc_trans; cg.Y = bufs->pc_list;
        cg.pd0 = (const float *)(ws + p.o_pd0); cg.pi0 = (const int *)(ws + p.o_pi0);
        cg.pd1 = (const float *)(ws + p.o_pd1); cg.pi1 = (const int *)(ws + p.o_pi1);
        cg.fx_bits = (const int *)(ws + p.o_fx);
        cg.N = N; cg.B = B; cg.S0 = S0; cg.S1 = p.S1; cg.G = G;
        cg.loss_part = (double *)(ws + p.o_floss);
        if (both) { cg.map = bufs->assign_map; cg.lambda = c.lambda_assign; cg.assign_part = (double *)(ws + p.o_apart); }
        g.has_cg = merged ? 0 : 1; g.cg_sl = (cg.S0 == 1 && cg.S1 == 1) ? 1 : ((cg.S0 <= 4 && cg.S1 <= 4) ? 4 : 0);
        if (merged) {
            PostArgs &pa = L.pa;
            pa.fl = fl; pa.cg = cg; pa.nfx = g.fgx; pa.nflow = pa.nfx * B; pa.ncx = g.ncg;
            pa.nwork = pa.nflow + g.ncg * B;
            const bool reorder = c.tune_reorder >= 0 && !g.static_order;
            for (int j = 0; j < 3; ++j) {
                const KnnJob &kj = j < 2 ? ka.job[j] : k3.job[0];
                pa.od.cost[j] = reorder ? kj.cost : nullptr;
                pa.od.border[j] = (int *)(ws + p.o_border) + (size_t)j * B * nqg;
            }
            pa.od.groups = B * nqg; pa.od.per = c.tune_xcd > 0 ? reart_div_up(B * nqg, 8) : B * nqg;
            pa.norder = reorder ? 3 : 0;
            g.post_blocks = pa.nwork + pa.norder;
            if (c.profile) {
                pa.od.prof = (const unsigned long long *)(ws + p.o_prof);
                pa.od.prof_pairs = (const unsigned int *)(ws + p.o_prof_pairs);
                pa.od.prof_acc = (unsigned long long *)(ws + p.o_prof_acc);
                pa.od.nprof = search_wgs;
                g.post_blocks += 1;
            }
        }
    }
    float *grads = (float *)(ws + p.o_grads);
    float *gW1 = grads, *gb1 = gW1 + 3 * H, *gW2 = gb1 + H, *g6d = gW2 + P * H, *gt = g6d + 6 * B * P;
    BaseBwdArgs &ba = L.ba;
    ba.cano = bufs->cano; ba.W1 = bufs->W1; ba.b1 = bufs->b1; ba.W2 = bufs->W2; ba.p6d = bufs->p6d; ba.pt = bufs->pt; ba.yT = fa.yT; ba.hT = fa.hT;
    ba.hard_idx = fa.hard_idx; ba.tau_ptr = bufs->tau; ba.tau = 1.0f; ba.G = G; ba.rt_table = fa.rt_table;
    ba.cano_idx = c.cano_idx;
    ba.gpf = c.use_flow ? (const float *)(ws + p.o_gpf) : nullptr;
    ba.cpts = c.tune_bwd_pts;
    ba.N = N; ba.P = P; ba.B = B; ba.H = H; ba.gW1 = gW1; ba.gb1 = gb1; ba.gW2 = gW2; ba.g6d = g6d; ba.gt = gt;
    FinalizeAdam &ad = L.ad;
    ad.enabled = 1; ad.W1 = bufs->W1; ad.b1 = bufs->b1; ad.W2 = bufs->W2; ad.p6d = bufs->p6d; ad.pt = bufs->pt;
    ad.m = bufs->adam_m; ad.v = bufs->adam_v; ad.seg_lr = c.seg_lr; ad.trans_lr = c.trans_lr;
    ad.beta1 = c.beta1; ad.beta2 = c.beta2; ad.eps = c.eps; ad.step_ptr = bufs->iter;
    ad.weight_decay = c.weight_decay;
    ad.step = (const float *)(ws + p.o_bc);
    ba.step_cur = (float *)(ws + p.o_bc); ba.step_next = ba.step_cur + 4;
    StepBook &bk = L.bk;
    bk.enabled = 1; bk.frame_loss = (const double *)(ws + p.o_floss); bk.n_frame_part = B * g.ncg;
    bk.flow_part = (const double *)(ws + p.o_fpart); bk.n_flow_part = nfp;
    bk.assign_part = both ? (const double *)(ws + p.o_apart) : nullptr; bk.n_assign_part = both ? B * g.ncg : 0;
    bk.losses_assign = bufs->losses_assign;
    bk.iter = bufs->iter; bk.tau = bufs->tau; bk.losses = bufs->losses; bk.step_next = (float *)(ws + p.o_bc) + 4;
    bk.ring = c.ring; bk.n_iter = c.n_iter; bk.lambda_flow = c.lambda_flow; bk.fixed_tau = c.fixed_tau;
    bk.end_tau = c.end_tau; bk.start_tau = c.start_tau; bk.beta1 = c.beta1; bk.beta2 = c.beta2;
    bk.seg_lr = c.seg_lr; bk.trans_lr = c.trans_lr;
    L.ws_bwd = ws + p.o_bwd; L.bwd_bytes = p.bwd_bytes;
    return REART_OK;
}

static bool step_batchable(const StepGeom &g) {
    return g.pruned && !g.static_order;
}

template <class A>
static Batched<A> gather(const StepLaunch *L, int K, A StepLaunch::*m) {
    Batched<A> b = {};
    for (int k = 0; k < K; ++k) b.a[k] = L[k].*m;
    return b;
}

static int step_launch(const StepLaunch *L, int K, hipStream_t st, hipEvent_t *ev, bool forward_only) {
    const StepGeom &g = L[0].g;
    if (K > 1 && !step_batchable(g)) return REART_ERR_UNSUPPORTED;
    MARK(0);
    int rc = reart_base_forward_launch(gather(L, K, &StepLaunch::fa).a, K, st, g.long_model);
    if (rc != REART_OK) return rc;
    MARK(1);
    if (forward_only) return REART_OK;
    const bool forked = !g.pruned && !ev && L[0].aux_stream && L[0].ev_fork && L[0].ev_join && g.flow;
    hipStream_t fst = forked ? (hipStream_t)L[0].aux_stream : st;
    if (forked) {
        if (hipEventRecord((hipEvent_t)L[0].ev_fork, st) != hipSuccess) return REART_ERR_LAUNCH;
        if (hipStreamWaitEvent(fst, (hipEvent_t)L[0].ev_fork, 0) != hipSuccess) return REART_ERR_LAUNCH;
    }
    if (g.has_search) {
        Batched<SearchArgs> sa = gather(L, K, &StepLaunch::sa);
        const int auto_s = K >= 3 ? 1 : (K == 2 ? 2 : 3);
        for (int k = 0; k < K; ++k) {
            if (L[k].auto_s1) sa.a[k].S1 = auto_s;
            if (L[k].auto_s3) sa.a[k].S3 = L[k].auto_s1 ? auto_s : sa.a[k].S1;
        }
        rc = K == 1 ? reart_search_launch(sa.a[0], st) : reart_search_launch_batch(sa.a, K, st);
        if (rc != REART_OK) return rc;
    } else if (!g.pruned && g.flow) {
        rc = g.grid ? reart_grid_query_launch(L[0].gq3, 3, fst) : reart_knn_launch_slices(L[0].k3, 3, fst);
        if (rc != REART_OK) return rc;
    }
    MARK(2);
    if (g.has_fl) {
        const dim3 fg(g.fgx, g.fgy, K);
        const Batched<FlowArgs> fb = gather(L, K, &StepLaunch::fl);
        if (K > 1) hipLaunchKernelGGL((flow_blend_kernel<1, true>), fg, dim3(FLOW_BS), 0, fst, fb);
        else if (g.fl_sl == 1) hipLaunchKernelGGL((flow_blend_kernel<1, false>), fg, dim3(FLOW_BS), 0, fst, fb);
        else if (g.fl_sl) hipLaunchKernelGGL((flow_blend_kernel<4, false>), fg, dim3(FLOW_BS), 0, fst, fb);
        else hipLaunchKernelGGL((flow_blend_kernel<0, false>), fg, dim3(FLOW_BS), 0, fst, fb);
        REART_CHECK_LAUNCH();
    }
    if (forked && hipEventRecord((hipEvent_t)L[0].ev_join, fst) != hipSuccess) return REART_ERR_LAUNCH;
    MARK(3);
    if (g.has_aa) {
        MARK(4);
        const dim3 ag(reart_div_up(g.N, CG_BS), g.B, K);
        const Batched<AssignArgs> ab = gather(L, K, &StepLaunch::aa);
        if (K > 1) hipLaunchKernelGGL(assign_grad_kernel<true>, ag, dim3(CG_BS), 0, st, ab);
        else hipLaunchKernelGGL(assign_grad_kernel<false>, ag, dim3(CG_BS), 0, st, ab);
    } else {
        if (!g.pruned) {
            if (g.grid) {
                rc = reart_grid_query_launch(L[0].gq1, 1, st);
                if (rc != REART_OK) return rc;
            }
            rc = reart_knn_launch_slices(L[0].ka, 1, st);
            if (rc != REART_OK) return rc;
        }
        MARK(4);
        if (g.merged) {
            const Batched<PostArgs> pb = gather(L, K, &StepLaunch::pa);
            static_assert(sizeof(Batched<PostArgs>) <= 3584, "kernel-argument segment");
            if (g.cg_assign) {
                if (K > 1) hipLaunchKernelGGL((post_kernel<true, true>), dim3(g.post_blocks, K), dim3(CG_BS), 0, st, pb);
                else hipLaunchKernelGGL((post_kernel<false, true>), dim3(g.post_blocks), dim3(CG_BS), 0, st, pb);
            } else if (K > 1) hipLaunchKernelGGL((post_kernel<true, false>), dim3(g.post_blocks, K), dim3(CG_BS), 0, st, pb);
            else hipLaunchKernelGGL((post_kernel<false, false>), dim3(g.post_blocks), dim3(CG_BS), 0, st, pb);
        } else {
            const dim3 cgd(g.ncg, g.B, K);
            const Batched<CGradArgs> cb = gather(L, K, &StepLaunch::cg);
            if (g.cg_assign) {
                if (K > 1) hipLaunchKernelGGL((chamfer_grad_kernel<1, true, true>), cgd, dim3(CG_BS), 0, st, cb);
                else if (g.cg_sl == 1) hipLaunchKernelGGL((chamfer_grad_kernel<1, false, true>), cgd, dim3(CG_BS), 0, st, cb);
                else if (g.cg_sl) hipLaunchKernelGGL((chamfer_grad_kernel<4, false, true>), cgd, dim3(CG_BS), 0, st, cb);
                else hipLaunchKernelGGL((chamfer_grad_kernel<0, false, true>), cgd, dim3(CG_BS), 0, st, cb);
            } else if (K > 1) hipLaunchKernelGGL((chamfer_grad_kernel<1, true, false>), cgd, dim3(CG_BS), 0, st, cb);
            else if (g.cg_sl == 1) hipLaunchKernelGGL((chamfer_grad_kernel<1, false, false>), cgd, dim3(CG_BS), 0, st, cb);
            else if (g.cg_sl) hipLaunchKernelGGL((chamfer_grad_kernel<4, false, false>), cgd, dim3(CG_BS), 0, st, cb);
            else hipLaunchKernelGGL((chamfer_grad_kernel<0, false, false>), cgd, dim3(CG_BS), 0, st, cb);
        }
    }
    REART_CHECK_LAUNCH();
    MARK(5);
    if (forked && hipStreamWaitEvent(st, (hipEvent_t)L[0].ev_join, 0) != hipSuccess) return REART_ERR_LAUNCH;
    const Batched<BaseBwdArgs> ba = gather(L, K, &StepLaunch::ba);
    const Batched<FinalizeAdam> ad = gather(L, K, &StepLaunch::ad);
    const Batched<StepBook> bk = gather(L, K, &StepLaunch::bk);
    const Batched<void *> wb = gather(L, K, &StepLaunch::ws_bwd);
    rc = reart_base_backward_launch(ba.a, ad.a, bk.a, wb.a, L[0].bwd_bytes, K, st, g.long_model);
    if (rc != REART_OK) return rc;
    MARK(6);
    MARK(7);
    MARK(8);
    return REART_OK;
}

static int relax_step_one(const reart_relax_config *cfg, const reart_relax_buffers *bufs, void *workspace, size_t workspace_bytes,
                          void *stream, hipEvent_t *ev, bool forward_only) {
    StepLaunch L;
    const int rc = step_describe(cfg, bufs, workspace, workspace_bytes, forward_only, &L);
    return rc != REART_OK ? rc : step_launch(&L, 1, (hipStream_t)stream, ev, forward_only);
}

extern "C" int reart_relax_step(const reart_relax_config *cfg, const reart_relax_buffers *bufs,
                                void *workspace, size_t workspace_bytes, void *stream) {
    return relax_step_one(cfg, bufs, workspace, workspace_bytes, stream, nullptr, false);
}

extern "C" int reart_relax_step_batch(const reart_relax_config *cfgs, const reart_relax_buffers *bufs, void *const *workspaces,
                                      size_t workspace_bytes, int K, void *stream) {
    if (!cfgs || !bufs || !workspaces || K < 1 || K > REART_BATCH_MAX) return REART_ERR_INVALID_ARG;
    static_assert(sizeof(Batched<SearchArgs>) <= 3584, "kernel-argument segment");
    StepLaunch L[REART_BATCH_MAX];
    for (int k = 0; k < K; ++k) {
        const int rc = step_describe(&cfgs[k], &bufs[k], workspaces[k], workspace_bytes, false, &L[k]);
        if (rc != REART_OK) return rc;
        if (!step_batchable(L[k].g)) return REART_ERR_UNSUPPORTED;
        if (memcmp(&L[k].g, &L[0].g, sizeof(StepGeom)) != 0 || L[k].bwd_bytes != L[0].bwd_bytes) return REART_ERR_INVALID_ARG;
    }
    return step_launch(L, K, (hipStream_t)stream, nullptr, false);
}

extern "C" int reart_relax_step_timed(const reart_relax_config *cfg, const reart_relax_buffers *bufs,
                                      void *workspace, size_t workspace_bytes, void *stream,
                                      float *h_ms) {
    if (!h_ms) return REART_ERR_INVALID_ARG;
    hipEvent_t ev[REART_RELAX_PHASES + 1];
    for (int k = 0; k <= REART_RELAX_PHASES; ++k)
        if (hipEventCreate(&ev[k]) != hipSuccess) return REART_ERR_LAUNCH;
    int rc = relax_step_one(cfg, bufs, workspace, workspace_bytes, stream, ev, false);
    if (rc == REART_OK) {
        if (hipEventSynchronize(ev[REART_RELAX_PHASES]) != hipSuccess) rc = REART_ERR_LAUNCH;
        for (int k = 0; k < REART_RELAX_PHASES && rc == REART_OK; ++k) {
            float ms = 0.f;
            if (hipEventElapsedTime(&ms, ev[k], ev[k + 1]) != hipSuccess) rc = REART_ERR_LAUNCH;
            h_ms[k] += ms;
        }
    }
    for (int k = 0; k <= REART_RELAX_PHASES; ++k) (void)hipEventDestroy(ev[k]);
    return rc;
}

extern "C" int reart_relax_profile(const reart_relax_config *cfg, void *workspace, size_t workspace_bytes,
                                   void *stream, double *h_out, int reset) {
    StepPlan p;
    if (!cfg || !h_out) return REART_ERR_INVALID_ARG;
    int rc = step_plan(cfg, &p);
    if (rc != REART_OK) return rc;
    if (!workspace || workspace_bytes < p.total) return REART_ERR_INVALID_ARG;
    if (!cfg->profile || !p.pruned) return REART_ERR_UNSUPPORTED;
    hipStream_t st = (hipStream_t)stream;
    unsigned long long acc[4] = {0, 0, 0, 0};
    if (hipMemcpyAsync(acc, (char *)workspace + p.o_prof_acc, sizeof(acc), hipMemcpyDeviceToHost, st) != hipSuccess ||
        hipStreamSynchronize(st) != hipSuccess)
        return REART_ERR_LAUNCH;
    int dev = 0, khz = 0;
    if (hipGetDevice(&dev) != hipSuccess || hipDeviceGetAttribute(&khz, hipDeviceAttributeWallClockRate, dev) != hipSuccess || khz <= 0)
        return REART_ERR_LAUNCH;
    const double hz = 1e3 * (double)khz;
    h_out[0] = (double)acc[0]; h_out[1] = (double)acc[1] / hz; h_out[2] = (double)acc[2]; h_out[3] = hz;
    h_out[4] = (double)acc[3] / hz;
    if (reset && hipMemsetAsync((char *)workspace + p.o_prof_acc, 0, sizeof(acc), st) != hipSuccess) return REART_ERR_LAUNCH;
    return REART_OK;
}

extern "C" int reart_relax_forward(const reart_relax_config *cfg, const reart_relax_buffers *bufs,
                                   void *workspace, size_t workspace_bytes, void *stream) {
    return relax_step_one(cfg, bufs, workspace, workspace_bytes, stream, nullptr, true);
}


__global__ void step_floor_init_kernel(int *chase, int n) {
    const int i = blockIdx.x * blockDim.x + threadIdx.x;
    if (i < n) chase[i] = (int)(((unsigned)i * 40503u + 12345u) % (unsigned)n);
}
__global__ void step_floor_kernel(const int *__restrict__ chase, int n, int loads, int barriers, int *sink) {
    extern __shared__ int fl_lds[];
    int idx = (int)((blockIdx.x * blockDim.x + threadIdx.x) % (unsigned)n);
    for (int l = 0; l < loads; ++l) idx = chase[idx];
    if (threadIdx.x == 0) fl_lds[0] = idx;
    for (int b_ = 0; b_ < barriers; ++b_) __syncthreads();
    if (idx < 0) sink[0] = fl_lds[0];
}
extern "C" int reart_relax_step_floor(const int *shape, int nk, int iters, void *workspace, size_t workspace_bytes, void *stream) {
    const int n = 16384;
    if (!shape || nk < 1 || nk > 8 || iters < 1 || !workspace || workspace_bytes < sizeof(int) * (size_t)n + 64) return REART_ERR_INVALID_ARG;
    for (int k = 0; k < nk; ++k)
        if (shape[5 * k] < 1 || shape[5 * k + 1] < 1 || shape[5 * k + 1] > 1024 || shape[5 * k + 2] < 4 || shape[5 * k + 2] > 64 * 1024 ||
            shape[5 * k + 3] < 0 || shape[5 * k + 4] < 0) return REART_ERR_INVALID_ARG;
    hipStream_t st = (hipStream_t)stream;
    int *chase = (int *)workspace, *sink = chase + n;
    hipLaunchKernelGGL(step_floor_init_kernel, dim3(n / 256), dim3(256), 0, st, chase, n);
    for (int it = 0; it < iters; ++it)
        for (int k = 0; k < nk; ++k)
            hipLaunchKernelGGL(step_floor_kernel, dim3(shape[5 * k]), dim3(shape[5 * k + 1]), (size_t)shape[5 * k + 2], st, chase, n,
                               shape[5 * k + 3], shape[5 * k + 4], sink);
    REART_CHECK_LAUNCH();
    return REART_OK;
}
```

Measured before the change: 13630 iterations/s.

## Pack search work items with query-frame index and hoist kernel args into scalar regs

Replaces the per-group border index array with packed item words that encode both the pair index and the query frame. The search kernel can then resolve qmap in a single uniform load instead of chained dependent global reads. KnnJob and SearchArgs are reordered so the hot fields sit in a compact head that is copied into scalar registers up front, and seed-point loads are issued before the LDS stores. Also adds profiling-only timestamp instrumentation that is compiled out by default. The packing only applies when the pair count and frame count fit in the bit budget; otherwise the old border path is used.

Measured after the change: 13890 iterations/s, median of 6. 1.02x the previous value.

```diff
diff --git a/reart_amd/csrc/internal.h b/reart_amd/csrc/internal.h
--- a/reart_amd/csrc/internal.h
+++ b/reart_amd/csrc/internal.h
@@ -117,20 +117,22 @@
 
 struct KnnJob {
     const float *q;
+    const float *q_alt;
     const float *tsoa;
+    const float *boxes;
+    const int *seed;
+    float *pd;
+    int *pi;
+    unsigned int *cost;
+    int P1, Ppad;
+    int nqg;
+    int P2;
+    const int *tlen;
+    const int *qmap;
+    int L;
     const int64_t *lenq;
     const int64_t *lent;
-    const float *q_alt;
-    const int *qmap;
-    const int *tlen;
-    const float *boxes;
-    const int *seed;
     const int *border;
-    unsigned int *cost;
-    int P1, P2, Ppad, L;
-    int nqg;
-    float *pd;
-    int *pi;
     float *dists;
     int64_t *idx;
 };
@@ -157,20 +159,33 @@
 #define NN_BOX 16
 #endif
 int reart_boxes_launch(const float *soa, int N, int Ppad, float *boxes, hipStream_t st);
+#define SEARCH_ITEM_PAIR_BITS 21
+#define SEARCH_ITEM_PAIR_MASK ((1u << SEARCH_ITEM_PAIR_BITS) - 1u)
+#if defined(__HIPCC__)
+#define REART_HD __host__ __device__
+#else
+#define REART_HD
+#endif
+REART_HD static inline bool reart_search_items_fit(long pairs, int frames) {
+    return pairs <= (long)SEARCH_ITEM_PAIR_MASK && frames + 1 < (1 << (32 - SEARCH_ITEM_PAIR_BITS));
+}
+REART_HD static inline unsigned int reart_search_item(int pair, int qb) { return (unsigned int)pair | ((unsigned int)(qb + 1) << SEARCH_ITEM_PAIR_BITS); }
 struct SearchArgs {
-    KnnJob k1[2]; int n1;
-    KnnJob k3;    int n3;
+    int n1, n3;
     int G;
     int per;
     int S1, S3;
+    int interleave;
     int sparse;
+    const unsigned int *item;
+    unsigned long long *prof;
+    unsigned int *prof_pairs;
     int share;
-    int interleave;
     int cloud_resident;
     int cloud_slices;
     int k_nqg;
-    unsigned long long *prof;
-    unsigned int *prof_pairs;
+    KnnJob k1[2];
+    KnnJob k3;
 };
 int reart_search_launch(const SearchArgs &a, hipStream_t st);
 int reart_search_launch_batch(const SearchArgs *a, int K, hipStream_t st);
diff --git a/reart_amd/csrc/prune.hip b/reart_amd/csrc/prune.hip
--- a/reart_amd/csrc/prune.hip
+++ b/reart_amd/csrc/prune.hip
@@ -2,8 +2,26 @@
 #include "internal.h"
 #include <math.h>
 #include <string.h>
+#include <stddef.h>
 
 typedef float f2 __attribute__((ext_vector_type(2)));
+struct SearchHot {
+    const float *q, *q_alt, *tsoa, *boxes;
+    const int *seed;
+    float *pd;
+    int *pi;
+    unsigned int *cost;
+    int P1, Ppad, nqg, P2;
+    const int *tlen;
+};
+static_assert(sizeof(SearchHot) == 88 && offsetof(KnnJob, tlen) == offsetof(SearchHot, tlen) && offsetof(KnnJob, q) == 0 && offsetof(KnnJob, q_alt) == offsetof(SearchHot, q_alt) &&
+              offsetof(KnnJob, tsoa) == offsetof(SearchHot, tsoa) && offsetof(KnnJob, boxes) == offsetof(SearchHot, boxes) &&
+              offsetof(KnnJob, seed) == offsetof(SearchHot, seed) && offsetof(KnnJob, pd) == offsetof(SearchHot, pd) &&
+              offsetof(KnnJob, pi) == offsetof(SearchHot, pi) && offsetof(KnnJob, cost) == offsetof(SearchHot, cost) &&
+              offsetof(KnnJob, P1) == offsetof(SearchHot, P1) && offsetof(KnnJob, Ppad) == offsetof(SearchHot, Ppad) &&
+              offsetof(KnnJob, nqg) == offsetof(SearchHot, nqg) && offsetof(KnnJob, P2) == offsetof(SearchHot, P2),
+              "SearchHot mirrors the head of KnnJob");
+__device__ __forceinline__ int pr_uniform_word(const void *p) { return *(const __attribute__((address_space(4))) int *)p; }
 #define PR_SMAX 4
 #define PR_QCAP 640
 #define PR_WPE 6
@@ -30,10 +48,30 @@
 #define PH_DECL unsigned long long ph_t = __builtin_amdgcn_s_memtime(), ph_acc[7] = {0, 0, 0, 0, 0, 0, 0}
 #define PH(k) do { const unsigned long long n_ = __builtin_amdgcn_s_memtime(); ph_acc[k] += n_ - ph_t; ph_t = n_; } while (0)
 #define PH_FLUSH(from, to) do { if ((threadIdx.x & 63) == 0) for (int k_ = from; k_ <= to; ++k_) atomicAdd(&g_prune_phase[k_], ph_acc[k_]); } while (0)
+__device__ unsigned long long g_prune_head[2][8];
+extern "C" int reart_debug_prune_head(unsigned long long *out, int reset) {
+    if (hipMemcpyFromSymbol(out, HIP_SYMBOL(g_prune_head), sizeof(g_prune_head)) != hipSuccess) return REART_ERR_LAUNCH;
+    if (reset) { unsigned long long z[16] = {0}; (void)hipMemcpyToSymbol(HIP_SYMBOL(g_prune_head), z, sizeof(z)); }
+    return REART_OK;
+}
+#define PH_HEAD_DECL unsigned long long hd_t = ph_t, hd_acc[3] = {0, 0, 0}
+#define PH_STAMP(k, ...) do { asm volatile("" :: __VA_ARGS__); const unsigned long long n_ = __builtin_amdgcn_s_memtime(); hd_acc[k] = n_ - hd_t; hd_t = n_; } while (0)
+#define PH_HEAD_FLUSH(row) do { if ((threadIdx.x & 63) == 0) { for (int k_ = 0; k_ < 3; ++k_) atomicAdd(&g_prune_head[row][1 + k_], hd_acc[k_]); \
+                                atomicAdd(&g_prune_head[row][4], ph_acc[0]); atomicAdd(&g_prune_head[row][6], 1ull); } } while (0)
+#define PH_ENTRY const unsigned long long hd_entry = __builtin_amdgcn_s_memtime(); unsigned long long hd_head = 0ull
+#define PH_HEAD_END do { hd_head = __builtin_amdgcn_s_memtime() - hd_entry; } while (0)
+#define PH_ENTRY_FLUSH(row) do { if ((threadIdx.x & 63) == 0) { atomicAdd(&g_prune_head[row][0], hd_head); \
+                                 atomicAdd(&g_prune_head[row][5], __builtin_amdgcn_s_memtime() - hd_entry); } } while (0)
 #else
 #define PH_DECL do { } while (0)
 #define PH(k) do { } while (0)
 #define PH_FLUSH(from, to) do { } while (0)
+#define PH_HEAD_DECL do { } while (0)
+#define PH_STAMP(k, ...) do { } while (0)
+#define PH_HEAD_FLUSH(row) do { } while (0)
+#define PH_ENTRY do { } while (0)
+#define PH_HEAD_END do { } while (0)
+#define PH_ENTRY_FLUSH(row) do { } while (0)
 #endif
 
 #define PR_WORK(w) ((unsigned)(w) << 20)
@@ -68,7 +106,8 @@
 }
 
 template <int KK, bool LDSV, int QCAP, bool BOXL>
-__device__ __forceinline__ void knn_pruned_wave(const KnnJob &jb, const int S, const int sparse, const int b, const int g,
+__device__ __forceinline__ void knn_pruned_wave(const float *qcloud, const int *seed_p, const int P1, const int n2,
+                                                const int S, const int sparse, const int b, const int g,
                                                 const int s, const float *cloud, const int cstride, const float *boxes_p,
                                                 float *s_tg, float *s_qc, unsigned int *s_q, float *s_bb, const int share, float *s_xthr,
                                                 unsigned long long *s_key, float &qx_o, float &qy_o, float &qz_o,
@@ -76,25 +115,25 @@
     struct { int S, sparse; } a = {S, sparse};
     const int lane = threadIdx.x & 63;
     PH_DECL;
+    PH_HEAD_DECL;
 
     const int i = g * NN_BS + lane;
-    const int ic = i < jb.P1 ? i : jb.P1 - 1;
-    const int qb = jb.qmap ? jb.qmap[b] : b;
-    const float *qp = (qb < 0 ? jb.q_alt : jb.q + (size_t)qb * jb.P1 * 3) + (size_t)ic * 3;
+    const int ic = i < P1 ? i : P1 - 1;
+    const float *qp = (const float *)((const char *)qcloud + 12u * (unsigned)ic);
     const float qx = qp[0], qy = qp[1], qz = qp[2];
+    PH_STAMP(0, "v"(qx), "v"(qy), "v"(qz));
     const f2 qx2 = {qx, qx}, qy2 = {qy, qy}, qz2 = {qz, qz};
 
     const float *tx = cloud;
     const float *ty = tx + cstride;
     const float *tz = ty + cstride;
-    const int n2 = jb.tlen ? jb.tlen[b] : jb.P2;
     const int nbox = (n2 + NN_BOX - 1) / NN_BOX;
     const float *bx = boxes_p;
 
     float thr = 0.f;
     unsigned int wp = 0u;
     {
-        const int *sd = jb.seed + ((size_t)b * jb.P1 + ic) * KK;
+        const int *sd = (const int *)((const char *)(seed_p + (size_t)b * P1 * KK) + 4u * KK * (unsigned)ic);
         int sj[KK];
         bool ok = true;
 #pragma unroll
@@ -104,17 +143,25 @@
 #pragma unroll
             for (int k2 = 0; k2 < k; ++k2) ok = ok && sj[k] != sj[k2];
         }
+        PH_STAMP(1, "v"(sj[0]), "v"(sj[KK - 1]), "s"(n2));
         constexpr bool SCR_JOINT = BOXL;
         constexpr bool SCR_FITS = (384 + QCAP + (SCR_JOINT ? 384 : 0)) >= KK * 3 * 64;
         if (SCR_FITS && share) {
             float *s_scr = (float *)s_key;
+            float sx[KK], sy[KK], sz[KK];
 #pragma unroll
             for (int k = 0; k < KK; ++k) {
                 const int j = ok ? sj[k] : 0;
-                s_scr[(3 * k + 0) * 64 + lane] = ok ? tx[j] : INFINITY;
-                s_scr[(3 * k + 1) * 64 + lane] = ok ? ty[j] : INFINITY;
-                s_scr[(3 * k + 2) * 64 + lane] = ok ? tz[j] : INFINITY;
-            }
+                sx[k] = tx[j]; sy[k] = ty[j]; sz[k] = tz[j];
+            }
+            if (!LDSV) __builtin_amdgcn_sched_barrier(0);
+#pragma unroll
+            for (int k = 0; k < KK; ++k) {
+                s_scr[(3 * k + 0) * 64 + lane] = ok ? sx[k] : INFINITY;
+                s_scr[(3 * k + 1) * 64 + lane] = ok ? sy[k] : INFINITY;
+                s_scr[(3 * k + 2) * 64 + lane] = ok ? sz[k] : INFINITY;
+            }
+            PH_STAMP(2, "v"(lane));
             thr = INFINITY;
             const float *row = s_scr + (lane & 48);
             const bool split = s_xthr != nullptr && a.S > 1;
@@ -389,6 +436,7 @@
     if (qcnt > 0) drain_queue();
     PH(5);
     PH_FLUSH(0, 5);
+    PH_HEAD_FLUSH(KK == 1 ? 0 : 1);
     qx_o = qx; qy_o = qy; qz_o = qz;
     work_o = (int)(wp >> 20); pairs_o = wp & 0xFFFFFu;
 }
@@ -396,7 +444,8 @@
 
 template <bool BATCH>
 __global__ __launch_bounds__(64 * PR_SMAX, PR_WPE) void knn_group_kernel(Batched<SearchArgs> ab) {
-    const SearchArgs &a = ab.a[BATCH ? blockIdx.y : 0];
+    PH_ENTRY;
+    const SearchArgs &a_ = ab.a[BATCH ? blockIdx.y : 0];
     extern __shared__ __attribute__((aligned(16))) unsigned char s_dyn[];
 #define PARK_M(t) ((float *)(s_dyn + (size_t)(t) * PR_LDS_WAVE_BYTES + 64 * 4 + 64 * 16))
 #define PARK_B(t) ((int *)(s_dyn + (size_t)(t) * PR_LDS_WAVE_BYTES + 64 * 4 + 64 * 16 + 3 * 64 * 4))
@@ -404,11 +453,13 @@
     __shared__ float s_xthr[PR_SMAX][64];
     __shared__ unsigned int s_ticket;
     __shared__ unsigned long long s_t0;
-    if (threadIdx.x == 0) { s_ticket = 0u; s_t0 = a.prof ? wall_clock64() : 0ull; }
-    __syncthreads();
+    struct { int n1, n3, G, per, S1, S3, interleave, sparse; } a = {a_.n1, a_.n3, a_.G, a_.per, a_.S1, a_.S3, a_.interleave, a_.sparse};
+    const unsigned int *const items = a_.item;
+    unsigned long long *const prof = a_.prof;
+    const int share = a_.share;
+    asm volatile("" :: "s"(a.n1), "s"(a.n3), "s"(a.G), "s"(a.per), "s"(a.S1), "s"(a.S3), "s"(a.interleave), "s"(a.sparse), "s"(items), "s"(prof), "s"(share));
     const int L = blockIdx.x, x = L & 7, r = L >> 3;
     const int s = threadIdx.x >> 6, lane = threadIdx.x & 63;
-    const unsigned long long t0 = s_t0;
     const int items1 = a.n1 * a.per, items3 = a.n3 * a.per;
     const int mixed = (a.n1 == 2 && a.n3) ? 3 * a.per : 0;
     int kind, idx;
@@ -426,15 +477,27 @@
     const int p = kind == 1 ? (a.n1 == 2 ? (idx >> 1) : idx) : idx;
     const int pos = a.interleave ? p * 8 + x : x * a.per + p;
     const bool live = p < a.per && pos < a.G && (kind == 1 ? idx < items1 : idx < items3);
+    const KnnJob *jp = kind == 1 ? &a_.k1[j] : &a_.k3;
+    int rec = pos;
+    if (items) rec = pr_uniform_word(items + ((size_t)(kind == 1 ? j : 2) * a.G + (live ? pos : 0)));
+    SearchHot h;
+    __builtin_memcpy(&h, jp, sizeof(SearchHot));
+    if (threadIdx.x == 0) { s_ticket = 0u; s_t0 = prof ? wall_clock64() : 0ull; }
+    __syncthreads();
+    asm volatile("" :: "s"(rec), "s"(h.tlen), "s"(h.q), "s"(h.q_alt), "s"(h.tsoa), "s"(h.boxes), "s"(h.seed), "s"(h.pd),
+                 "s"(h.pi), "s"(h.cost), "s"(h.P1), "s"(h.Ppad), "s"(h.nqg), "s"(h.P2));
+    const unsigned long long t0 = s_t0;
     if (!live) {
-        if (a.prof && threadIdx.x == 0) { a.prof[2 * (size_t)L] = t0; a.prof[2 * (size_t)L + 1] = t0; a.prof_pairs[L] = 0u; }
+        if (prof && threadIdx.x == 0) { prof[2 * (size_t)L] = t0; prof[2 * (size_t)L + 1] = t0; a_.prof_pairs[L] = 0u; }
         return;
     }
-    const KnnJob &jb = kind == 1 ? a.k1[j] : a.k3;
     const int S = kind == 1 ? a.S1 : a.S3;
     if (s >= S) return;
-    const int grp = jb.border ? jb.border[pos] : pos;
-    const int b = grp / jb.nqg, g = grp - b * jb.nqg;
+    const int grp = items ? (int)((unsigned)rec & SEARCH_ITEM_PAIR_MASK) : (jp->border ? jp->border[pos] : pos);
+    const int b = grp / h.nqg, g = grp - b * h.nqg;
+    const int qb = items ? (int)((unsigned)rec >> SEARCH_ITEM_PAIR_BITS) - 1 : (jp->qmap ? jp->qmap[b] : b);
+    const int n2 = h.tlen ? pr_uniform_word(h.tlen + b) : h.P2;
+    const float *qcloud = qb < 0 ? h.q_alt : h.q + (size_t)qb * h.P1 * 3;
     float qx = 0.f, qy = 0.f, qz = 0.f;
     float bm[3] = {INFINITY, INFINITY, INFINITY};
     int bb[3] = {-1, -1, -1};
@@ -451,17 +514,19 @@
         float *s_bb = (float *)s_q;
         s_q += 384;
         constexpr int QC = PR_QCAP - 384;
-        const float *cloud = jb.tsoa + (size_t)b * 3 * jb.Ppad;
-        const float *boxes_p = jb.boxes + (size_t)b * (jb.Ppad / NN_BOX) * 8;
+        const float *cloud = h.tsoa + (size_t)b * 3 * h.Ppad;
+        const float *boxes_p = h.boxes + (size_t)b * (h.Ppad / NN_BOX) * 8;
+        PH_HEAD_END;
         if (kind == 1) {
             float m1[1]; int b1[1];
-            knn_pruned_wave<1, false, QC, true>(jb, S, a.sparse, b, g, s, cloud, jb.Ppad, boxes_p, s_tg, s_qc, s_q, s_bb, a.share, a.share > 1 ? &s_xthr[0][0] : nullptr, s_key,
+            knn_pruned_wave<1, false, QC, true>(qcloud, h.seed, h.P1, n2, S, a.sparse, b, g, s, cloud, h.Ppad, boxes_p, s_tg, s_qc, s_q, s_bb, share, share > 1 ? &s_xthr[0][0] : nullptr, s_key,
                                                qx, qy, qz, m1, b1, work, pairs);
             bm[0] = m1[0]; bb[0] = b1[0];
         } else {
-            knn_pruned_wave<3, false, QC, true>(jb, S, a.sparse, b, g, s, cloud, jb.Ppad, boxes_p, s_tg, s_qc, s_q, s_bb, a.share, a.share > 1 ? &s_xthr[0][0] : nullptr, s_key,
+            knn_pruned_wave<3, false, QC, true>(qcloud, h.seed, h.P1, n2, S, a.sparse, b, g, s, cloud, h.Ppad, boxes_p, s_tg, s_qc, s_q, s_bb, share, share > 1 ? &s_xthr[0][0] : nullptr, s_key,
                                                qx, qy, qz, bm, bb, work, pairs);
         }
+        PH_ENTRY_FLUSH(kind == 1 ? 0 : 1);
     }
     if (S > 1) {
 #pragma unroll
@@ -482,7 +547,7 @@
         for (int k = 0; k < 3; ++k) { bm[k] = PARK_M(0)[k * 64 + lane]; bb[k] = PARK_B(0)[k * 64 + lane]; }
     }
     const int i = g * NN_BS + lane;
-    const float *tx = jb.tsoa + (size_t)b * 3 * jb.Ppad, *ty = tx + jb.Ppad, *tz = ty + jb.Ppad;
+    const float *tx = h.tsoa + (size_t)b * 3 * h.Ppad, *ty = tx + h.Ppad, *tz = ty + h.Ppad;
     if (kind == 1) {
         float m = bm[0];
         int blk = bb[0];
@@ -501,9 +566,9 @@
             }
         }
         pairs += 64u * (NN_BOX / 2);
-        if (i < jb.P1) {
-            const size_t o = (size_t)b * jb.P1 + i;
-            jb.pd[o] = m; jb.pi[o] = bi;
+        if (i < h.P1) {
+            const size_t o = (size_t)b * h.P1 + i;
+            h.pd[o] = m; h.pi[o] = bi;
         }
     } else {
         float kd[3] = {INFINITY, INFINITY, INFINITY};
@@ -517,17 +582,17 @@
                 reart_top3_insert(kd, ki, PARK_M(t)[k * 64 + lane], bt >= 0 ? bt : 0x7fffffff);
             }
         }
-        if (i < jb.P1) {
-            const size_t o = ((size_t)b * jb.P1 + i) * 3;
-#pragma unroll
-            for (int k = 0; k < 3; ++k) { jb.pd[o + k] = kd[k]; jb.pi[o + k] = kd[k] < INFINITY ? ki[k] : -1; }
+        if (i < h.P1) {
+            const size_t o = ((size_t)b * h.P1 + i) * 3;
+#pragma unroll
+            for (int k = 0; k < 3; ++k) { h.pd[o + k] = kd[k]; h.pi[o + k] = kd[k] < INFINITY ? ki[k] : -1; }
         }
     }
     if (lane == 0) {
-        if (jb.cost) jb.cost[pos] = (unsigned int)work;
-        if (a.prof) {
-            a.prof[2 * (size_t)L] = t0; a.prof[2 * (size_t)L + 1] = wall_clock64();
-            a.prof_pairs[L] = pairs;
+        if (h.cost) h.cost[pos] = (unsigned int)work;
+        if (prof) {
+            prof[2 * (size_t)L] = t0; prof[2 * (size_t)L + 1] = wall_clock64();
+            a_.prof_pairs[L] = pairs;
         }
     }
 }
@@ -573,13 +638,16 @@
         unsigned char *wl = wbase + (size_t)w * PC_WAVE_BYTES;
         float *s_qc = (float *)wl;
         unsigned int *s_q = (unsigned int *)(wl + 64 * 16 + 3 * 64 * 8);
+        const int qb = jb.qmap ? jb.qmap[b] : b;
+        const float *qcloud = qb < 0 ? jb.q_alt : jb.q + (size_t)qb * jb.P1 * 3;
+        const int n2 = jb.tlen ? jb.tlen[b] : jb.P2;
         if (kind == 1) {
             float m1[1]; int b1[1];
-            knn_pruned_wave<1, true, PC_QCAP, false>(jb, S, a.sparse, b, g, sl, cl, Ppad, bxs, nullptr, s_qc, s_q, nullptr, a.share, nullptr, s_key, qx, qy, qz,
+            knn_pruned_wave<1, true, PC_QCAP, false>(qcloud, jb.seed, jb.P1, n2, S, a.sparse, b, g, sl, cl, Ppad, bxs, nullptr, s_qc, s_q, nullptr, a.share, nullptr, s_key, qx, qy, qz,
                                               m1, b1, work, pairs);
             bm[0] = m1[0]; bb[0] = b1[0];
         } else {
-            knn_pruned_wave<3, true, PC_QCAP, false>(jb, S, a.sparse, b, g, sl, cl, Ppad, bxs, nullptr, s_qc, s_q, nullptr, a.share, nullptr, s_key, qx, qy, qz,
+            knn_pruned_wave<3, true, PC_QCAP, false>(qcloud, jb.seed, jb.P1, n2, S, a.sparse, b, g, sl, cl, Ppad, bxs, nullptr, s_qc, s_q, nullptr, a.share, nullptr, s_key, qx, qy, qz,
                                               bm, bb, work, pairs);
         }
         if (S > 1 && sl > 0) {
diff --git a/reart_amd/csrc/step.hip b/reart_amd/csrc/step.hip
--- a/reart_amd/csrc/step.hip
+++ b/reart_amd/csrc/step.hip
@@ -21,7 +21,7 @@
     int W1, W3;
     int sparse;
     size_t o_seed3;
-    size_t o_border;
+    size_t o_item;
     size_t o_cost;
     size_t o_prof, o_prof_pairs, o_prof_acc;
     size_t o_gridY, o_gridR;
@@ -88,7 +88,7 @@
     p->o_boxR = ws.take_bytes(sizeof(float) * 8 * (size_t)c->B * (p->Mpad / NN_BOX + 1));
     p->o_seed3 = ws.take_bytes((p->pruned && c->use_flow) ? sizeof(int) * BN * 3 : 0);
     const size_t G = (size_t)c->B * reart_div_up(c->N, NN_BS);
-    p->o_border = ws.take_bytes(sizeof(int) * 3 * G);
+    p->o_item = ws.take_bytes(sizeof(unsigned int) * 3 * G);
     p->o_cost = ws.take_bytes(sizeof(unsigned int) * 3 * G);
     const size_t nprof = (c->profile && p->pruned) ? (size_t)reart_search_grid(2, 1, (int)G) : 0;
     p->o_prof = ws.take_bytes(sizeof(unsigned long long) * 2 * nprof);
@@ -112,7 +112,7 @@
                                   int *__restrict__ rlen, int *__restrict__ qmap,
                                   int64_t *__restrict__ iter, float *__restrict__ tau,
                                   const float *__restrict__ pc_list, int *__restrict__ fx_bits,
-                                  float *__restrict__ adam_step, int *__restrict__ seed3, int *__restrict__ border) {
+                                  float *__restrict__ adam_step, int *__restrict__ seed3, unsigned int *__restrict__ item) {
     __shared__ float s_max[1024];
     const int t = threadIdx.x;
     if (seed3)
@@ -131,13 +131,16 @@
         fx_bits[0] = bits > 39 ? 39 : (bits < 0 ? 0 : bits);
     }
     if (t < c.B) {
+        const int qm = (t < c.cano_idx) ? t : (t == c.cano_idx ? -1 : t - 1);
+        qmap[t] = qm;
+        if (c.use_flow) rlen[t] = ref_off[t + 1] - ref_off[t];
         {
             const int nqg = (c.N + NN_BS - 1) / NN_BS, ng = c.B * nqg;
+            const bool words = reart_search_items_fit((long)ng, c.B);
             for (int g = 0; g < nqg; ++g)
-                for (int j = 0; j < 3; ++j) border[j * ng + t * nqg + g] = t * nqg + g;
-        }
-        qmap[t] = (t < c.cano_idx) ? t : (t == c.cano_idx ? -1 : t - 1);
-        if (c.use_flow) rlen[t] = ref_off[t + 1] - ref_off[t];
+                for (int j = 0; j < 3; ++j)
+                    item[j * ng + t * nqg + g] = words ? reart_search_item(t * nqg + g, j < 2 ? t : qm) : (unsigned int)(t * nqg + g);
+        }
     }
     if (t == 0) {
         const long it = (long)iter[0];
@@ -191,7 +194,7 @@
     hipLaunchKernelGGL(relax_init_kernel, dim3(1), dim3(1024), 0, st, *cfg, bufs->ref_off,
                        (int *)(ws + p.o_rlen), (int *)(ws + p.o_qmap), bufs->iter, bufs->tau, bufs->pc_list,
                        (int *)(ws + p.o_fx), (float *)(ws + p.o_bc),
-                       (p.pruned && cfg->use_flow) ? (int *)(ws + p.o_seed3) : nullptr, (int *)(ws + p.o_border));
+                       (p.pruned && cfg->use_flow) ? (int *)(ws + p.o_seed3) : nullptr, (unsigned int *)(ws + p.o_item));
     if (hipMemsetAsync(ws + p.o_ticket, 0, 4 * sizeof(unsigned int), st) != hipSuccess) return REART_ERR_LAUNCH;
     if (hipMemsetAsync(ws + p.o_prof_acc, 0, 4 * sizeof(unsigned long long), st) != hipSuccess) return REART_ERR_LAUNCH;
     if (p.pruned) {
@@ -461,7 +464,7 @@
 }
 struct OrderArgs {
     const unsigned int *cost[3];
-    int *border[3];
+    unsigned int *item[3];
     int groups;
     int per;
     const unsigned long long *prof; const unsigned int *prof_pairs; unsigned long long *prof_acc; int nprof;
@@ -473,14 +476,15 @@
     if (!o.cost[j] || o.groups > ORD_MAX * CG_BS) return;
     for (int e = tid; e < 8 * 256; e += CG_BS) s_hist[e] = 0u;
     __syncthreads();
-    int old[ORD_MAX], bucket[ORD_MAX];
+    unsigned int old[ORD_MAX];
+    int bucket[ORD_MAX];
 #pragma unroll
     for (int u = 0; u < ORD_MAX; ++u) {
         const int k = tid + u * CG_BS;
-        old[u] = 0; bucket[u] = -1;
+        old[u] = 0u; bucket[u] = -1;
         if (k < o.groups) {
             const unsigned int c = o.cost[j][k] >> 5;
-            old[u] = o.border[j][k];
+            old[u] = o.item[j][k];
             bucket[u] = (k / o.per) * 256 + 255 - (int)(c < 255u ? c : 255u);
             atomicAdd(&s_hist[bucket[u]], 1u);
         }
@@ -504,7 +508,7 @@
     __syncthreads();
 #pragma unroll
     for (int u = 0; u < ORD_MAX; ++u)
-        if (bucket[u] >= 0) o.border[j][atomicAdd(&s_hist[bucket[u]], 1u)] = old[u];
+        if (bucket[u] >= 0) o.item[j][atomicAdd(&s_hist[bucket[u]], 1u)] = old[u];
 }
 __device__ __forceinline__ void prof_body(const OrderArgs &o) {
     __shared__ unsigned long long s_lo[CG_BS / 64], s_hi[CG_BS / 64], s_sum[CG_BS / 64], s_busy[CG_BS / 64];
@@ -658,6 +662,7 @@
 
     const int nqg = reart_div_up(N, NN_BS);
     const int *qmap = (const int *)(ws + p.o_qmap);
+    const bool item_words = reart_search_items_fit((long)B * nqg, B);
     KnnArgs &ka = L.ka, &k3 = L.k3;
     ka.N = B; ka.S = p.S1; ka.K = 1; ka.euclidean = 0;
     for (int j = 0; j < 2; ++j) {
@@ -669,7 +674,7 @@
         kj.pi = (int *)(ws + (j == 0 ? p.o_pi0 : p.o_pi1));
         kj.boxes = c.use_boxes ? (const float *)(ws + (j == 0 ? p.o_boxY : p.o_boxX)) : nullptr;
         kj.seed = p.pruned ? kj.pi : nullptr;
-        kj.border = (const int *)(ws + p.o_border) + (size_t)j * B * nqg;
+        kj.border = item_words ? nullptr : (const int *)(ws + p.o_item) + (size_t)j * B * nqg;
         kj.cost = p.pruned ? (unsigned int *)(ws + p.o_cost) + (size_t)j * B * nqg : nullptr;
     }
     ka.items0 = B * nqg * p.S1; ka.items = 2 * ka.items0;
@@ -682,7 +687,7 @@
         kj.P1 = N; kj.P2 = c.M_max; kj.Ppad = p.Mpad; kj.L = p.Mpad / p.S3; kj.nqg = nqg;
         kj.pd = (float *)(ws + p.o_pd3); kj.pi = (int *)(ws + p.o_pi3);
         kj.seed = p.pruned ? (const int *)(ws + p.o_seed3) : nullptr;
-        kj.border = (const int *)(ws + p.o_border) + 2 * (size_t)B * nqg;
+        kj.border = item_words ? nullptr : (const int *)(ws + p.o_item) + 2 * (size_t)B * nqg;
         kj.cost = p.pruned ? (unsigned int *)(ws + p.o_cost) + 2 * (size_t)B * nqg : nullptr;
         k3.job[1] = kj;
         k3.items0 = B * nqg * p.S3; k3.items = k3.items0;
@@ -697,6 +702,7 @@
     int search_wgs = 0, S3 = p.S3, S0 = p.S1;
     if (p.pruned) {
         SearchArgs &sa = L.sa;
+        sa.item = item_words ? (const unsigned int *)(ws + p.o_item) : nullptr;
         sa.G = B * nqg; sa.S1 = p.W1; sa.S3 = p.W3; sa.sparse = p.sparse; sa.share = c.tune_share < 0 ? 0 : (c.tune_share == 1 ? 1 : 2); sa.interleave = c.tune_xcd > 0 ? 0 : 1;
         sa.cloud_resident = c.tune_cloud > 0 ? 1 : 0; sa.cloud_slices = c.tune_cloud > 0 ? c.tune_cloud : 0;
         if (chamfer) { sa.k1[0] = ka.job[0]; sa.k1[1] = ka.job[1]; sa.n1 = 2; }
@@ -770,7 +776,7 @@
             for (int j = 0; j < 3; ++j) {
                 const KnnJob &kj = j < 2 ? ka.job[j] : k3.job[0];
                 pa.od.cost[j] = reorder ? kj.cost : nullptr;
-                pa.od.border[j] = (int *)(ws + p.o_border) + (size_t)j * B * nqg;
+                pa.od.item[j] = (unsigned int *)(ws + p.o_item) + (size_t)j * B * nqg;
             }
             pa.od.groups = B * nqg; pa.od.per = c.tune_xcd > 0 ? reart_div_up(B * nqg, 8) : B * nqg;
             pa.norder = reorder ? 3 : 0;
```
